# srvk/eesen

Measured on AMD Instinct MI355X. Metric: CTC training frames/sec (whole node), 4x512 BiLSTM, higher is better.
Workload: dtype f32

## Files before the change

### eesen_amd/csrc/kernels.h

```cpp
#pragma once
#include "common.h"

namespace eesen {

struct GemmBound {
  const float* p = nullptr;
  int per_index = 0;
};
void gemm_f32(hipStream_t st, bool a_kc, bool b_kc, int M, int N, int K, float alpha, const float* A, int lda,
              const float* B, int ldb, float beta, float* C, int ldc, const float* bias, float* ws,
              size_t ws_floats, int extra_lds_bytes = 0,
              bool bf16_operands = false,
              GemmBound bound_a = {}, GemmBound bound_b = {});

constexpr int kDefaultGemmMode = 2;
int gemm_mode();
void set_gemm_mode(int mode);
void amax_abs(hipStream_t st, const float* P, long rows, int cols, int ld, float* out);
void amax_abs_accumulate(hipStream_t st, const float* P, long rows, int cols, int ld, float* out);
constexpr int kAmaxBlocks = 512;
void amax_rows_cols(hipStream_t st, const float* P, long rows, int cols, int ld, float* out_rows, float* out_cols, float* ws);

#ifndef EESEN_SHARDS
#define EESEN_SHARDS 8
#endif
constexpr int kShards = EESEN_SHARDS, kShardStride = 32;
constexpr int kCtlHalf = 2048 * kShards;

struct GemmGate {
  const unsigned* cnt;
  unsigned* err;
  int ndir, nz, nblk;
  int T, S;
  int spin_limit;
};
void gemm_f32_nt_gated(hipStream_t st, int M, int N, int K, const float* A, int lda, const float* B, int ldb, float* C,
                       int ldc, const float* bias, const GemmGate& gate, GemmBound bound_a = {}, GemmBound bound_b = {});

struct LstmLayerDev {
  int T, S, H, ndir;
  float* G;
  float* C;
  float* Y;
  float* X = nullptr;
  const float* Wm;
  const float* WmT;
  const float* peep;
  const int* lens;
  const float* rmask = nullptr;
  int drop_mode = 0;
  int s_begin = 0, s_count = 0;
  float* PX = nullptr;
  size_t px_floats = 0;
  int poll_delay = 0;
  int poll_raw = 0;
  unsigned* milestone = nullptr;
  int milestone_step = 0;
  int xcd_map = 1, fwd_mux = 1, bwd_q4 = 1, bwd_ksplit = 1, bwd_mux = 1;
  int fwd_t16_small = 1;
  int fwd_narrow2 = 1;
  int bwd_q4_st8 = 1;
  int fwd_bf16 = 0;
  int fwd_split = 0;
  int fwd_f16 = 0;
  const float* wm_amax = nullptr;
  int bwd_f16 = 0;
  unsigned char* DGH = nullptr;
  float* EX = nullptr;
};
float handoff_flight_ns();
void set_gpu_share(int n);
int gpu_share_value();
void wait_for_word(hipStream_t st, const unsigned* word, unsigned target, unsigned* err, double limit_s = 2.0);
void lstm_fwd_step(hipStream_t st, const LstmLayerDev& L, int step);
void lstm_bwd_step(hipStream_t st, const LstmLayerDev& L, int step, const float* dY, int lddy, float* DG, float* DCF);
void dropout_mask(hipStream_t st, float* out, long rows, int cols, int ld, float p, unsigned long long seed, bool per_column);
void activation_rows(hipStream_t st, bool tanh_, const float* x, int ldx, float* y, int ldy, long rows, int cols);
void activation_diff_rows(hipStream_t st, bool tanh_, const float* y, int ldy, float* d, int ldd, long rows, int cols);
void mul_elements(hipStream_t st, const float* a, int lda, const float* m, int ldm, float* out, int ldo, long rows, int cols);
enum { kRecNone = 0, kRecFwdBf = 1, kRecFwdMux = 2, kRecFwdF32 = 3, kRecBwdQ4 = 4, kRecBwdKsplit = 5, kRecBwdKsplitMux = 6, kRecBwdGeneric = 7 };
struct RecPlan {
  int kind = kRecNone;
  const char* kernel = "";
  int seq_tile = 0;
  int units = 0;
  int windows = 0;
  int grid[3] = {0, 0, 0};
  int wgs = 0;
  int wgs_per_cu = 0;
  int vgprs = 0, lds = 0;
  int free_vgprs = -1;
  int seq_tiles = 1;
  bool one_window = false;
  bool leaves_room = false;
  bool bf16 = false;
  bool light = false;
  size_t need_px = 0, need_ex = 0;
  bool need_dgh = false;
  size_t ctl_words = 0;
  int chunk = 0;
  const void* fn = nullptr;
};
RecPlan lstm_fwd_plan(const LstmLayerDev& L);
RecPlan lstm_bwd_plan(const LstmLayerDev& L);
void lstm_fwd_launch(hipStream_t st, const RecPlan& plan, const LstmLayerDev& L, unsigned* cnt, unsigned* err, int spin_limit,
                     unsigned long long* trace = nullptr, hipEvent_t after_reset = nullptr);
void lstm_bwd_launch(hipStream_t st, const RecPlan& plan, const LstmLayerDev& L, const float* dY, int lddy, float* DG, unsigned* cnt,
                     unsigned* err, int spin_limit, unsigned long long* trace = nullptr);
void lstm_bias_peep_grads(hipStream_t st, const LstmLayerDev& L, const float* DG, float* bias_grad, float* peep_grad,
                          float* ws, size_t ws_floats);
size_t lstm_bias_peep_ws_floats(int T, int S, int H, int ndir);

void col_sums(hipStream_t st, const float* M, int rows, int cols, int ld, float* out, float* ws, size_t ws_floats);
size_t col_sums_ws_floats(int rows, int cols);

void softmax_rows(hipStream_t st, const float* x, int ldx, float* y, int ldy, int rows, int K);
void log_rows(hipStream_t st, const float* in, int ldi, float* out, int ldo, int rows, int K);
void ctc_alpha_beta(hipStream_t st, const float* logp, int ld, int T, int S, int Lpad, const int* labx, const int* lens,
                    const int* lablens, float* alpha, float* beta, float* pzx, int waves = 0);
int ctc_sweep_waves(int Lpad, int waves = 0);
void ctc_best_path(hipStream_t st, const float* scores, int ld, int T, int S, int Lpad, const int* labx, const int* lens,
                   const int* lablens, float* delta, int waves = 0);
void ctc_traceback(hipStream_t st, const float* delta, int T, int S, int Lpad, const int* labx, const int* lens, const int* lablens,
                   int* ali, int* pos, float* score);
void ctc_row_topc(hipStream_t st, const float* scores, int ld, int rows, int K, int S, const int* lens, int Cc, int* cid, float* csc,
                  float* sblank);
struct LmTables;
struct LexTables;
void ctc_prefix_beam(hipStream_t st, const float* scores, int ld, int T, int S, const int* lens, int B, int Cc, const int* cid,
                     const float* csc, const float* sblank, const LmTables* lm, const LexTables* lex, float alpha, float beta, bool use_eos,
                     int* tparent, int* tlabel, int* fnode, int* flen, float* fscore, float* flm, int* count);
void ctc_hyp(hipStream_t st, const int* tparent, const int* tlabel, const int* fnode, const int* flen, const float* fscore, const float* flm,
             const int* count, int T, int S, int B, int N, int* hyp, int* hyp_len, float* score, float* lm_out);
struct WordLexTables;
void ctc_word_beam(hipStream_t st, const float* scores, int ld, int T, int S, const int* lens, int B, int Cc, const int* cid,
                   const float* csc, const float* sblank, const LmTables* lm, const WordLexTables& lex, float alpha, float beta, bool use_eos,
                   int* tparent, int* tlabel, int* tword, int* fnode, int* flen, float* fscore, float* flm, int* fword, int* fnw, int* count);
void ctc_word_hyp(hipStream_t st, const int* tparent, const int* tlabel, const int* tword, const int* fnode, const int* flen, const float* fscore,
                  const float* flm, const int* fword, const int* fnw, const int* count, int T, int S, int B, int N, int* hyp, int* hyp_len,
                  float* score, float* lm_out, int* words, int* ends, int* word_len);
void ctc_error_diff(hipStream_t st, const float* probs, int ld, int T, int S, int K, int Lpad, int Lmax, const int* lens,
                    const int* lablens, const int* labx, const float* alpha, const float* beta,
                    const float* pzx, float* diff, int ldd);
void log_sub_prior(hipStream_t st, float* m, int ld, int rows, int K, bool apply_log, const float* log_prior, float prior_scale);
void row_argmax(hipStream_t st, const float* m, int ld, int rows, int K, int* ids);

struct CeSums {
  double obj;
  long long correct;
};
int ce_eval_blocks(int rows);
void ce_eval(hipStream_t st, const float* y, int ld, int rows, int K, int S, const int* lens, const int* tgt, float* diff,
             int ldd, CeSums* part, CeSums* out);

void sgd_update(hipStream_t st, float* param, float* corr, const float* fresh, long n, float mmt, float lr_coef,
                float max_grad, const unsigned* skip = nullptr, const float* live = nullptr);
void zero_if_set(hipStream_t st, float* p, long n, const unsigned* word);
void adaptive_update(hipStream_t st, float* param, float* corr, const float* fresh, float* accu, long n, float mmt, float lr,
                     float max_grad, float eps, float rho, float one_minus_rho, bool rmsprop, const unsigned* skip = nullptr,
                     const float* live = nullptr);
void tensor_moments(hipStream_t st, const float* base, long rows, int cols, long ld, double* out6, double* ws,
                    int nb = 0, int hf = 0, int hi = 0);
void transpose2d(hipStream_t st, const float* src, int rows, int cols, float* dst);
void copy2d(hipStream_t st, const float* src, int lds, float* dst, int ldd, int rows, int cols);

}
```

### eesen_amd/csrc/net.cpp

```cpp
#include "net.h"

#include <algorithm>
#include <cmath>
#include <cstdio>
#include <cstring>

namespace eesen {


int PhaseTimer::begin(hipStream_t st, int phase) {
  if (!on_) return -1;
  if (used_ == spans_.size()) spans_.emplace_back();
  spans_[used_].phase = phase;
  spans_[used_].a.record(st);
  return (int)used_++;
}
void PhaseTimer::end(hipStream_t st, int idx) {
  if (!on_ || idx < 0) return;
  spans_[idx].b.record(st);
}
void PhaseTimer::collect(float* out, int nphase) {
  for (int i = 0; i < nphase; ++i) out[i] = 0.f;
  for (size_t i = 0; i < used_; ++i) {
    spans_[i].b.wait();
    float ms = 0.f;
    EESEN_HIP_CHECK(hipEventElapsedTime(&ms, spans_[i].a, spans_[i].b));
    if (spans_[i].phase >= 0 && spans_[i].phase < nphase) out[spans_[i].phase] += ms * 1e-3f;
  }
  if (accumulate_) used_ = 0;
}

int PhaseTimer::spans(int* phases, float* secs, int cap) {
  for (size_t i = 0; i < used_ && (int)i < cap; ++i) {
    spans_[i].b.wait();
    float ms = 0.f;
    EESEN_HIP_CHECK(hipEventElapsedTime(&ms, spans_[i].a, spans_[i].b));
    if (phases) phases[i] = spans_[i].phase;
    if (secs) secs[i] = ms * 1e-3f;
  }
  return (int)used_;
}

long Layer::file_params() const {
  if (is_lstm()) return (long)ndir * ((long)4 * Hf * din_f + (long)4 * Hf * Hf + 4 * Hf + 3 * Hf);
  if (kind == EESEN_LAYER_AFFINE) return (long)dout_f * din_f + dout_f;
  return 0;
}

const char* Layer::marker() const {
  switch (kind) {
    case EESEN_LAYER_BILSTM_PARALLEL: return nonparallel ? "<BiLstm>" : "<BiLstmParallel>";
    case EESEN_LAYER_LSTM_PARALLEL: return nonparallel ? "<Lstm>" : "<LstmParallel>";
    case EESEN_LAYER_AFFINE: return "<AffineTransform>";
    case EESEN_LAYER_SOFTMAX: return "<Softmax>";
    case EESEN_LAYER_SIGMOID: return "<Sigmoid>";
    case EESEN_LAYER_TANH: return "<Tanh>";
  }
  return "<Unknown>";
}

template <class F>
static void for_each_param(const Layer& L, F f) {
  long fi = 0;
  if (L.is_lstm()) {
    const int H = L.H, Hf = L.Hf, D = L.din_f, D4 = pad4(L.din);
    for (int dir = 0; dir < L.ndir; ++dir) {
      for (int r = 0; r < 4 * Hf; ++r) {
        const int q = r / Hf, u = r % Hf;
        for (int d = 0; d < D; ++d) f(fi++, L.off_wx + ((size_t)dir * 4 * H + u * 4 + q) * D4 + L.in_col(d));
      }
      for (int r = 0; r < 4 * Hf; ++r) {
        const int q = r / Hf, u = r % Hf;
        for (int k = 0; k < Hf; ++k) f(fi++, L.off_wm + ((size_t)dir * 4 * H + u * 4 + q) * H + k);
      }
      for (int r = 0; r < 4 * Hf; ++r) f(fi++, L.off_bias + (size_t)dir * 4 * H + (r % Hf) * 4 + r / Hf);
      for (int g = 0; g < 3; ++g)
        for (int u = 0; u < Hf; ++u) f(fi++, L.off_peep + ((size_t)dir * 3 + g) * H + u);
    }
  } else if (L.kind == EESEN_LAYER_AFFINE) {
    const int D4 = pad4(L.din);
    for (int r = 0; r < L.dout; ++r)
      for (int d = 0; d < L.din_f; ++d) f(fi++, L.off_w + (size_t)r * D4 + L.in_col(d));
    for (int r = 0; r < L.dout; ++r) f(fi++, L.off_b + r);
  }
}

Net::Net(int dev, void* stream) : device(dev) {
  require_device(dev);
  st = reinterpret_cast<hipStream_t>(stream);
  int lo = 0, hi = 0;
  EESEN_HIP_CHECK(hipDeviceGetStreamPriorityRange(&lo, &hi));
  EESEN_HIP_CHECK(hipStreamCreateWithPriority(&st2.s, hipStreamNonBlocking, lo));
  tn = Tuning::from_env();
  persistent = tn.persistent;
  gate_fwd = tn.gate_fwd >= 0 ? tn.gate_fwd != 0 : gemm_mode() == 0;
  overlap = tn.overlap >= 0 ? tn.overlap != 0 : persistent != 0;
  spin_limit = tn.spin_limit;
  if (tn.trace) {
    trace.reserve(1280);
    EESEN_HIP_CHECK(hipMemset(trace.p, 0, 1280 * sizeof(unsigned long long)));
  }
  ctl.reserve(kCtlWords);
  EESEN_HIP_CHECK(hipMemset(ctl.p, 0, kCtlWords * sizeof(unsigned)));
  {
    constexpr float kFwdNs = 400.f, kBwdNs = 280.f, kBwdSideNs = 420.f, kRefFlightNs = 400.f;
    flight_ns = handoff_flight_ns();
    const float fscale = flight_ns >= 300.f && flight_ns <= 700.f ? 1.f : flight_ns / kRefFlightNs;
    auto ticks = [&](float ns) { return std::min(300, std::max(0, (int)std::lround(fscale * ns / 10.f))); };
    delay_fwd = ticks(kFwdNs); delay_bwd = ticks(kBwdNs); delay_bwd_side = ticks(kBwdSideNs);
    if (const char* e = tn.poll_ns) {
      int a = -1, b2 = -1;
      if (sscanf(e, "%d,%d", &a, &b2) == 2) { delay_fwd = a / 10; delay_bwd = delay_bwd_side = b2 / 10; poll_raw = 1; }
    }
    if (tn.print_flight)
      fprintf(stderr, "eesen_hip: increment flight %.0f ns; first-poll delays forward %d0, backward %d0 (beside side-stream GEMMs %d0) ns\n", flight_ns, delay_fwd, delay_bwd, delay_bwd_side);
  }
}

Net::~Net() {
  (void)hipSetDevice(device);
  (void)hipStreamSynchronize(st);
  for (StatGuard* g : guards) {
    (void)hipStreamSynchronize(g->st);
    g->word = nullptr;
    g->net = nullptr;
  }
  if (trace.p) {
    std::vector<unsigned long long> h(1280);
    if (hipMemcpy(h.data(), trace.p, h.size() * 8, hipMemcpyDeviceToHost) == hipSuccess)
      for (int pass = 0; pass < 2; ++pass) {
        double seg[5] = {0, 0, 0, 0, 0};
        int n = 0;
        for (int s = 8; s < 120; ++s) {
          const unsigned long long* a = h.data() + pass * 640 + s * 5;
          if (!a[0] || !a[5]) continue;
          seg[0] += (double)(a[1] - a[0]); seg[1] += (double)(a[2] - a[1]); seg[2] += (double)(a[3] - a[2]);
          seg[3] += (double)(a[4] - a[3]); seg[4] += (double)(a[5] - a[4]);
          ++n;
        }
        if (n) fprintf(stderr, "EESEN_TRACE %s: wait %.0f | A-load+MFMA+reduce %.0f | epilogue %.0f | drain+barrier %.0f | publish->next %.0f ticks/step (%d steps)\n",
                       pass ? "bwd" : "fwd", seg[0] / n, seg[1] / n, seg[2] / n, seg[3] / n, seg[4] / n, n);
      }
  }
  if (st2) (void)hipStreamSynchronize(st2);
}

void StatGuard::hook(Net* n, int device, hipStream_t stream, const char* entry_point) {
  if (n && !(n->device == device && n->st == stream))
    throw Error(EESEN_ERR_INVALID, std::string(entry_point) + ": the loss object and the Net must live on the same device and stream");
  unhook();
  if (!n || !n->ctl.p) return;
  word = n->ctl.p + kCtlWords - 1;
  net = n;
  st = stream;
  n->guards.push_back(this);
}

void StatGuard::unhook() {
  if (net) net->guards.erase(std::remove(net->guards.begin(), net->guards.end(), this), net->guards.end());
  word = nullptr;
  net = nullptr;
}

void StatGuard::note_dropped(const char* what) {
  if (dropped++ == 0 || dropped % 100 == 0)
    fprintf(stderr, "WARNING (eesen_hip) %s statistics of a minibatch computed from a timed-out forward pass were dropped (%ld so far)\n", what, dropped);
}

void Net::sync() {
  EESEN_HIP_CHECK(hipSetDevice(device));
  EESEN_HIP_CHECK(hipStreamSynchronize(st));
  wait_buckets_host();
  comm_check_alive(comm);
  check_device_error(true);
}

void Net::check_device_error(bool consumer) {
  if (!ctl.p) return;
  unsigned e = 0;
  EESEN_HIP_CHECK(hipMemcpy(&e, ctl.p + kCtlWords - 1, sizeof(unsigned), hipMemcpyDeviceToHost));
  if (!e) { steps_since_clean = 0; return; }
  EESEN_HIP_CHECK(hipStreamSynchronize(st));
  EESEN_HIP_CHECK(hipMemset(ctl.p + kCtlWords - 1, 0, sizeof(unsigned)));
  const bool only_waiter = e == 2 && tn.fwd_mid;
  if (only_waiter) tn.fwd_mid = 0;
  else { persistent = 0; gate_fwd = false; overlap = false; }
  ++recoveries;
  const int lost = std::max(1, steps_since_clean);
  steps_since_clean = 0;
  const bool rerun = consumer && propagated && input.p && rows > 0;
  const char* what = comm ? "contributed a ZERO gradient to the data-parallel sum (the ranks' models stay identical)" : "were NOT applied";
  if (only_waiter)
    fprintf(stderr, "WARNING (eesen_hip) the side stream's wait for a forward-recurrence milestone gave up (kernels serialised by a tool?): "
                    "%d minibatch(es) in flight %s%s; continuing without the early input GEMM (EESEN_FWD_MID=0)\n", lost, what,
            rerun ? " and the last forward pass is re-run" : "");
  else
    fprintf(stderr, "WARNING (eesen_hip) a persistent recurrence kernel gave up waiting for a peer workgroup (GPU shared or preempted?): "
                    "%d minibatch(es) in flight %s%s; continuing with the one-launch-per-step kernels\n", lost, what,
            rerun ? " and the last forward pass is re-run" : "");
  if (rerun) {
    forward_pass();
    EESEN_HIP_CHECK(hipStreamSynchronize(st));
  }
}

void Net::arm_device_error_poll() {
  if (!ctl.p) return;
  if (!err_pin.p) *static_cast<unsigned*>(err_pin.reserve(sizeof(unsigned))) = 0;
  EESEN_HIP_CHECK(hipMemcpyAsync(err_pin.p, ctl.p + kCtlWords - 1, sizeof(unsigned), hipMemcpyDeviceToHost, st));
  err_pin.used(st);
  err_armed = true;
}

void Net::poll_device_error() {
  if (!err_armed || !err_pin.ev.query()) return;
  err_armed = false;
  if (*err_pin.as<unsigned>()) check_device_error(false);
  else steps_since_clean = 0;
}

void Net::add_layer(int kind, int din, int dout, float coef, float max_grad) {
  EESEN_REQUIRE(!finalized, EESEN_ERR_STATE, "net already finalized");
  EESEN_REQUIRE(din > 0 && dout > 0, EESEN_ERR_INVALID, "layer dimensions must be positive");
  const Layer* prev = layers.empty() ? nullptr : &layers.back();
  if (prev)
    EESEN_REQUIRE(prev->dout_f == din, EESEN_ERR_INVALID, "Dimensionality mismatch between consecutive layers");
  Layer L;
  L.kind = kind; L.coef = coef; L.max_grad = max_grad;
  L.din_f = din; L.dout_f = dout;
  L.din = prev ? prev->dout : din;
  if (prev) { L.in_nb = prev->out_nb; L.in_hf = prev->out_hf; L.in_hi = prev->out_hi; }
  L.dout = dout;
  const char* sees_pad = "directly on an LSTM layer whose cell count per direction is not a multiple of 4 is not supported: it would see the "
                         "zero cells the library pads such a layer with";
  switch (kind) {
    case EESEN_LAYER_BILSTM_PARALLEL:
      EESEN_REQUIRE(dout % 2 == 0, EESEN_ERR_INVALID, "<CellDim> of a BiLstm layer must be even");
      L.ndir = 2; L.Hf = dout / 2;
      break;
    case EESEN_LAYER_LSTM_PARALLEL:
      L.ndir = 1; L.Hf = dout;
      break;
    case EESEN_LAYER_AFFINE:
      break;
    case EESEN_LAYER_SOFTMAX:
      EESEN_REQUIRE(din == dout, EESEN_ERR_INVALID, "Softmax needs InputDim == OutputDim");
      if (L.in_nb) throw Error(EESEN_ERR_INVALID, std::string("a <Softmax> ") + sees_pad);
      break;
    case EESEN_LAYER_SIGMOID:
    case EESEN_LAYER_TANH:
      EESEN_REQUIRE(din == dout, EESEN_ERR_INVALID, "an activation layer needs InputDim == OutputDim");
      if (L.in_nb && kind == EESEN_LAYER_SIGMOID) throw Error(EESEN_ERR_INVALID, std::string("a <Sigmoid> ") + sees_pad + " (sigmoid(0) = 1/2)");
      L.dout = L.din;
      L.out_nb = L.in_nb; L.out_hf = L.in_hf; L.out_hi = L.in_hi;
      break;
    default:
      throw Error(EESEN_ERR_INVALID, "unsupported layer kind " + std::to_string(kind));
  }
  if (L.is_lstm()) {
    L.H = pad4(L.Hf);
    L.dout = L.ndir * L.H;
    if (L.H != L.Hf) { L.out_nb = L.ndir; L.out_hf = L.Hf; L.out_hi = L.H; }
  }
  layers.push_back(std::move(L));
}

void Net::finalize() {
  EESEN_REQUIRE(!finalized, EESEN_ERR_STATE, "net already finalized");
  EESEN_REQUIRE(!layers.empty(), EESEN_ERR_INVALID, "empty net");
  EESEN_HIP_CHECK(hipSetDevice(device));
  size_t off = 0;
  for (Layer& L : layers) {
    L.p_off = off;
    size_t n = 0;
    if (L.is_lstm()) {
      const size_t H = L.H, D4 = pad4(L.din), nd = L.ndir;
      L.off_wx = n;   n += nd * 4 * H * D4;
      L.off_bias = n; n += nd * 4 * H;
      L.off_wm = n;   n += nd * 4 * H * H;
      L.off_peep = n; n += nd * 3 * H;
      L.WmT.reserve(nd * H * 4 * H);
    } else if (L.kind == EESEN_LAYER_AFFINE) {
      L.off_w = n; n += (size_t)L.dout * pad4(L.din);
      L.off_b = n; n += pad4(L.dout);
    }
    L.p_n = (n + 3) & ~(size_t)3;
    off += L.p_n;
  }
  P = off;
  if (P) {
    params.reserve(P); corr.reserve(P); fresh.reserve(P + kLiveWords);
    EESEN_HIP_CHECK(hipMemsetAsync(params.p, 0, P * sizeof(float), st));
    EESEN_HIP_CHECK(hipMemsetAsync(corr.p, 0, P * sizeof(float), st));
    EESEN_HIP_CHECK(hipMemsetAsync(fresh.p, 0, (P + kLiveWords) * sizeof(float), st));
  }
  if (tn.overlap < 0)
    for (const Layer& L : layers)
      if (L.is_lstm() && L.H > 512) overlap = false;
  amax.reserve(1 + layers.size());
  EESEN_HIP_CHECK(hipMemsetAsync(amax.p, 0, amax.cap * sizeof(float), st));
  EESEN_HIP_CHECK(hipMemsetD32Async(reinterpret_cast<hipDeviceptr_t>(amax.p), 0x3f800000, 1, st));
  finalized = true;
  refresh_derived();
  sync();
}

void Net::measure(const float* Pm, long nrows, int cols, int ld, DevBuf<float>& out_rows, DevBuf<float>& out_cols) {
  out_rows.reserve((size_t)nrows);
  out_cols.reserve((size_t)cols);
  amax_ws.reserve((size_t)kAmaxBlocks * std::min(16384, (cols + 3) & ~3));
  amax_rows_cols(st, Pm, nrows, cols, ld, out_rows.p, out_cols.p, amax_ws.p);
}
bool Net::x_is_bounded(int li) const {
  if (li == 0) return false;
  const Layer& Pv = layers[li - 1];
  return (Pv.is_lstm() && !Pv.cur_fwd_drop) || Pv.is_activation() || Pv.kind == EESEN_LAYER_SOFTMAX;
}
void Net::ensure_weight_amax() {
  const bool mode2 = gemm_mode() == 2;
  const bool need_w = mode2 && !wamax_valid;
  if (wm_valid && !need_w) return;
  if (!wm_valid) EESEN_HIP_CHECK(hipMemsetAsync(am_wm(0), 0, layers.size() * sizeof(float), st));
  for (size_t li = 0; li < layers.size(); ++li) {
    Layer& L = layers[li];
    if (L.is_lstm()) {
      if (need_w) measure(params.p + L.p_off + L.off_wx, (long)L.ndir * 4 * L.H, pad4(L.din), pad4(L.din), L.bw.rows, L.bw.cols);
      if (!wm_valid) amax_abs_accumulate(st, params.p + L.p_off + L.off_wm, (long)L.ndir * 4 * L.H, L.H, L.H, am_wm((int)li));
    } else if (L.kind == EESEN_LAYER_AFFINE && need_w) measure(params.p + L.p_off + L.off_w, L.dout, pad4(L.din), pad4(L.din), L.bw.rows, L.bw.cols);
  }
  wm_valid = true;
  if (mode2) wamax_valid = true;
}

long Net::num_params() const {
  long n = 0;
  for (const Layer& L : layers) n += L.file_params();
  return n;
}

void Net::init_accu() {
  if (accu_init) return;
  accu.reserve(P);
  EESEN_HIP_CHECK(hipMemsetAsync(accu.p, 0, P * sizeof(float), st));
  accu_init = true;
}

void Net::refresh_derived() {
  wamax_valid = wm_valid = false;
  for (Layer& L : layers)
    if (L.is_lstm())
      for (int dir = 0; dir < L.ndir; ++dir)
        transpose2d(st, params.p + L.p_off + L.off_wm + (size_t)dir * 4 * L.H * L.H, 4 * L.H, L.H,
                    L.WmT.p + (size_t)dir * L.H * 4 * L.H);
}

int Net::tensor_moments(int which, int layer, double* out6_host, int cap_tensors) {
  EESEN_REQUIRE(finalized, EESEN_ERR_STATE, "net not finalized");
  EESEN_REQUIRE(layer >= 0 && layer < (int)layers.size(), EESEN_ERR_INVALID, "layer index out of range");
  EESEN_REQUIRE(which >= 0 && which <= 2, EESEN_ERR_INVALID, "which: 0 parameters, 1 momentum buffers, 2 accumulators");
  const Layer& L = layers[layer];
  struct Region { size_t off; long rows; int cols; long ld; int nb, hf, hi; };
  std::vector<Region> reg;
  if (L.is_lstm()) {
    const int H = L.H, Hf = L.Hf, D4 = pad4(L.din);
    for (int dir = 0; dir < L.ndir; ++dir) {
      reg.push_back({L.off_wx + (size_t)dir * 4 * H * D4, 4L * Hf, L.din_f, D4, L.in_nb, L.in_hf, L.in_hi});
      reg.push_back({L.off_wm + (size_t)dir * 4 * H * H, 4L * Hf, Hf, H, 0, 0, 0});
      reg.push_back({L.off_bias + (size_t)dir * 4 * H, 1, 4 * Hf, 4L * H, 0, 0, 0});
      for (int g = 0; g < 3; ++g) reg.push_back({L.off_peep + ((size_t)dir * 3 + g) * H, 1, Hf, H, 0, 0, 0});
    }
  } else if (L.kind == EESEN_LAYER_AFFINE) {
    reg.push_back({L.off_w, L.dout, L.din_f, pad4(L.din), L.in_nb, L.in_hf, L.in_hi});
    reg.push_back({L.off_b, 1, L.dout, L.dout, 0, 0, 0});
  }
  const int n = (int)reg.size();
  if (!out6_host || n == 0) return n;
  EESEN_REQUIRE(cap_tensors >= n, EESEN_ERR_INVALID, "moments buffer too small");
  EESEN_HIP_CHECK(hipSetDevice(device));
  if (which == 2) init_accu();
  sync();
  const float* base = (which == 0 ? params.p : which == 1 ? corr.p : accu.p) + L.p_off;
  DevBuf<double> d;
  d.reserve((size_t)n * 6 + 8);
  for (int i = 0; i < n; ++i)
    eesen::tensor_moments(st, base + reg[i].off, reg[i].rows, reg[i].cols, reg[i].ld, d.p + (size_t)i * 6, d.p + (size_t)n * 6, reg[i].nb, reg[i].hf, reg[i].hi);
  EESEN_HIP_CHECK(hipStreamSynchronize(st));
  EESEN_HIP_CHECK(hipMemcpy(out6_host, d.p, (size_t)n * 6 * sizeof(double), hipMemcpyDeviceToHost));
  return n;
}

static void upload_flat(Net& net, DevBuf<float>& dst, const float* host, long n) {
  EESEN_REQUIRE(net.finalized, EESEN_ERR_STATE, "net not finalized");
  EESEN_REQUIRE(n == net.num_params(), EESEN_ERR_INVALID, "parameter count mismatch");
  EESEN_HIP_CHECK(hipSetDevice(net.device));
  std::vector<float> h(net.P, 0.f);
  long base = 0;
  for (const Layer& L : net.layers) {
    for_each_param(L, [&](long fi, size_t io) { h[L.p_off + io] = host[base + fi]; });
    base += L.file_params();
  }
  net.sync();
  if (net.P) EESEN_HIP_CHECK(hipMemcpy(dst.p, h.data(), net.P * sizeof(float), hipMemcpyHostToDevice));
}

void Net::set_params(const float* host, long n) {
  upload_flat(*this, params, host, n);
  refresh_derived();
  sync();
}

void Net::set_accu(const float* host, long n) {
  init_accu();
  upload_flat(*this, accu, host, n);
}

void Net::get_flat(const DevBuf<float>& buf, float* host, long n) {
  EESEN_REQUIRE(finalized, EESEN_ERR_STATE, "net not finalized");
  EESEN_REQUIRE(n == num_params(), EESEN_ERR_INVALID, "parameter count mismatch");
  sync();
  std::vector<float> h(P);
  if (P) EESEN_HIP_CHECK(hipMemcpy(h.data(), buf.p, P * sizeof(float), hipMemcpyDeviceToHost));
  long base = 0;
  for (const Layer& L : layers) {
    for_each_param(L, [&](long fi, size_t io) { host[base + fi] = h[L.p_off + io]; });
    base += L.file_params();
  }
}

void Net::set_seq_lengths(const int* l, int s) {
  EESEN_REQUIRE(s > 0, EESEN_ERR_INVALID, "need at least one sequence");
  EESEN_HIP_CHECK(hipSetDevice(device));
  lens.assign(l, l + s);
  for (int v : lens) EESEN_REQUIRE(v >= 0, EESEN_ERR_INVALID, "negative sequence length");
  poll_device_error();
  lens_d.reserve(s);
  int* pinned = static_cast<int*>(lens_pin.reserve(s * sizeof(int), std::max<size_t>(64, (size_t)s * 2) * sizeof(int)));
  std::copy(lens.begin(), lens.end(), pinned);
  EESEN_HIP_CHECK(hipMemcpyAsync(lens_d.p, pinned, s * sizeof(int), hipMemcpyHostToDevice, st));
  lens_pin.used(st);
  S = s;
  propagated = false;
}

static LstmLayerDev lstm_view(const Net& net, const Layer& L, int T) {
  LstmLayerDev d;
  d.T = T; d.S = net.S; d.H = L.H; d.ndir = L.ndir;
  d.G = L.G.p; d.C = L.C.p; d.Y = L.Y.p;
  d.X = L.X.p;
  d.Wm = net.params.p + L.p_off + L.off_wm;
  d.WmT = L.WmT.p;
  d.peep = net.params.p + L.p_off + L.off_peep;
  d.lens = net.lens_d.p;
  d.rmask = L.cur_drop_mode ? L.rmask.p : nullptr;
  d.drop_mode = L.cur_drop_mode;
  d.fwd_bf16 = net.fwd_bf16_rec ? 1 : 0;
  d.fwd_split = net.tn.fwd_split;
  d.fwd_f16 = net.tn.fwd_f16 && net.tn.fwd_split;
  d.bwd_f16 = net.tn.bwd_f16 && net.tn.fwd_split;
  d.wm_amax = net.amax.p ? const_cast<Net&>(net).am_wm((int)(&L - net.layers.data())) : nullptr;
  d.xcd_map = net.tn.xcd_map; d.fwd_mux = net.tn.fwd_mux; d.bwd_q4 = net.tn.bwd_q4; d.bwd_q4_st8 = net.tn.bwd_q4_st8; d.fwd_narrow2 = net.tn.fwd_narrow2; d.fwd_t16_small = net.tn.fwd_t16_small; d.bwd_ksplit = net.tn.bwd_ksplit; d.bwd_mux = net.tn.bwd_mux;
  return d;
}

void Net::set_layer_dropout(int layer, const float* nine) {
  EESEN_REQUIRE(layer >= 0 && layer < (int)layers.size(), EESEN_ERR_INVALID, "layer index out of range");
  Layer& L = layers[layer];
  bool any = false;
  for (int k = 0; k < 9; ++k) any |= nine[k] != 0.f;
  EESEN_REQUIRE(!any || L.kind == EESEN_LAYER_BILSTM_PARALLEL, EESEN_ERR_INVALID, "dropout options exist on BiLstm layers only");
  EESEN_REQUIRE(nine[0] >= 0.f && nine[0] < 1.f && nine[7] >= 0.f && nine[7] < 1.f, EESEN_ERR_INVALID, "dropout factor outside [0, 1)");
  for (int k = 0; k < 9; ++k) L.drop[k] = (k == 0 || k == 7) ? nine[k] : (nine[k] != 0.f ? 1.f : 0.f);
}

void Net::get_layer_dropout(int layer, float* nine) const {
  EESEN_REQUIRE(layer >= 0 && layer < (int)layers.size(), EESEN_ERR_INVALID, "layer index out of range");
  for (int k = 0; k < 9; ++k) nine[k] = layers[layer].drop[k];
}

static void widen_mask(const Layer& L, const float* src, long n, std::vector<float>& dst, const char* what) {
  dst.clear();
  if (!src) return;
  const long wf = (long)L.ndir * L.Hf, wi = (long)L.ndir * L.H;
  EESEN_REQUIRE(n > 0 && n % wf == 0, EESEN_ERR_INVALID, std::string(what) + ": the float count is not a multiple of the layer's ndir * H columns");
  if (wf == wi) { dst.assign(src, src + n); return; }
  const long rows = n / wf;
  dst.assign((size_t)rows * wi, 0.f);
  for (long r = 0; r < rows; ++r)
    for (int d = 0; d < L.ndir; ++d)
      std::copy(src + r * wf + (long)d * L.Hf, src + r * wf + (long)(d + 1) * L.Hf, dst.begin() + r * wi + (long)d * L.H);
}

void Net::set_dropout_masks(int layer, const float* fwd, long fwd_n, const float* rec, int rec_rows, long rec_n, int coin) {
  EESEN_REQUIRE(layer >= 0 && layer < (int)layers.size() && layers[layer].is_lstm(), EESEN_ERR_INVALID, "not an LSTM layer");
  Layer& L = layers[layer];
  if (rec) EESEN_REQUIRE(rec_rows > 0 && rec_n == (long)rec_rows * L.ndir * L.Hf, EESEN_ERR_INVALID, "recurrent mask: rec_floats must be rec_rows x ndir * H");
  widen_mask(L, fwd, fwd ? fwd_n : 0, L.inj_fmask, "forward mask");
  widen_mask(L, rec, rec ? rec_n : 0, L.inj_rmask, "recurrent mask");
  L.inj_rmask_rows = rec ? rec_rows : 0;
  L.inj_coin = coin;
}

void Net::get_dropout_masks(int layer, float* fwd_host, float* rec_host, int* info4) {
  EESEN_REQUIRE(layer >= 0 && layer < (int)layers.size() && layers[layer].is_lstm(), EESEN_ERR_INVALID, "not an LSTM layer");
  EESEN_REQUIRE(propagated, EESEN_ERR_STATE, "no Propagate yet");
  Layer& L = layers[layer];
  EESEN_HIP_CHECK(hipSetDevice(device));
  sync();
  const size_t ldY = (size_t)L.ndir * L.H, wf = (size_t)L.ndir * L.Hf;
  auto fetch = [&](float* host, const float* dev, size_t nrows) {
    if (wf == ldY) { EESEN_HIP_CHECK(hipMemcpy(host, dev, nrows * ldY * sizeof(float), hipMemcpyDeviceToHost)); return; }
    std::vector<float> tmp(nrows * ldY);
    EESEN_HIP_CHECK(hipMemcpy(tmp.data(), dev, tmp.size() * sizeof(float), hipMemcpyDeviceToHost));
    for (size_t r = 0; r < nrows; ++r)
      for (int d = 0; d < L.ndir; ++d)
        std::copy(tmp.begin() + r * ldY + (size_t)d * L.H, tmp.begin() + r * ldY + (size_t)d * L.H + L.Hf, host + r * wf + (size_t)d * L.Hf);
  };
  if (fwd_host && L.cur_fwd_drop) fetch(fwd_host, L.fmask.p, (size_t)rows);
  if (rec_host && L.cur_drop_mode) fetch(rec_host, L.rmask.p, (size_t)(T + 2) * S);
  if (info4) { info4[0] = L.cur_fwd_drop; info4[1] = L.cur_drop_mode; info4[2] = L.cur_twiddle_coin; info4[3] = (int)wf; }
}

static void prepare_dropout(Net& net, Layer& L) {
  L.cur_fwd_drop = false; L.cur_drop_mode = 0; L.cur_twiddle_coin = false;
  const bool want = net.in_train && L.has_dropout();
  if (!want) { L.inj_fmask.clear(); L.inj_rmask.clear(); L.inj_rmask_rows = 0; L.inj_coin = -1; return; }
  const float fwd_p = L.drop[0], rec_p = L.drop[7];
  const bool fw_seq = L.drop[2] != 0.f, rec_step = L.drop[3] != 0.f, rec_seq = L.drop[4] != 0.f;
  const bool rnndrop = L.drop[5] != 0.f, nml = L.drop[6] != 0.f, twiddle = L.drop[8] != 0.f;
  const int T = net.T, S = net.S, ldY = L.ndir * L.H;
  bool coin = false;
  if (twiddle) {
    if (L.inj_coin >= 0) coin = L.inj_coin != 0;
    else {
      unsigned long long z = net.drop_seed + (++net.drop_counter) * 0x9E3779B97F4A7C15ull;
      z = (z ^ (z >> 30)) * 0xBF58476D1CE4E5B9ull; z = (z ^ (z >> 27)) * 0x94D049BB133111EBull; z ^= z >> 31;
      coin = (z >> 63) != 0;
    }
  }
  L.cur_twiddle_coin = coin;
  const bool rec = (rnndrop || nml) && (!twiddle || !coin);
  const bool fwd = fwd_p > 0.f && (!twiddle || coin);
  if (rec) {
    EESEN_REQUIRE(rec_step != rec_seq, EESEN_ERR_INVALID,
                  "recurrent dropout needs exactly one of RecurrentTimeStepDropout / RecurrentSequenceDropout (bilstm-layer.h:102-113)");
    EESEN_REQUIRE(!(rnndrop && nml), EESEN_ERR_INVALID, "RNNDrop and NoMemLossDropout are mutually exclusive");
    const long mrows = (long)(T + 2) * S;
    L.rmask.reserve((size_t)mrows * ldY);
    if (!L.inj_rmask.empty()) {
      EESEN_REQUIRE((L.inj_rmask_rows == mrows || L.inj_rmask_rows == S) && (long)L.inj_rmask.size() == (long)L.inj_rmask_rows * ldY,
                    EESEN_ERR_INVALID, "injected recurrent mask has the wrong shape");
      const size_t chunk = (size_t)L.inj_rmask_rows * ldY;
      for (long r0 = 0; r0 < mrows; r0 += L.inj_rmask_rows)
        EESEN_HIP_CHECK(hipMemcpyAsync(L.rmask.p + (size_t)r0 * ldY, L.inj_rmask.data(), chunk * sizeof(float), hipMemcpyHostToDevice, net.st));
      EESEN_HIP_CHECK(hipStreamSynchronize(net.st));
    } else {
      dropout_mask(net.st, L.rmask.p, mrows, ldY, ldY, rec_p, net.drop_seed + (++net.drop_counter) * 0x632BE59BD9B4E019ull, rec_seq);
    }
    L.cur_drop_mode = rnndrop ? 2 : 1;
  }
  if (fwd) {
    L.fmask.reserve((size_t)net.rows * ldY);
    L.Yd.reserve((size_t)net.rows * ldY);
    if (!L.inj_fmask.empty()) {
      EESEN_REQUIRE((long)L.inj_fmask.size() == (long)net.rows * ldY, EESEN_ERR_INVALID, "injected forward mask has the wrong shape");
      EESEN_HIP_CHECK(hipMemcpyAsync(L.fmask.p, L.inj_fmask.data(), L.inj_fmask.size() * sizeof(float), hipMemcpyHostToDevice, net.st));
      EESEN_HIP_CHECK(hipStreamSynchronize(net.st));
    } else {
      dropout_mask(net.st, L.fmask.p, net.rows, ldY, ldY, fwd_p, net.drop_seed + (++net.drop_counter) * 0x632BE59BD9B4E019ull, fw_seq);
    }
    L.cur_fwd_drop = true;
  }
  L.inj_fmask.clear(); L.inj_rmask.clear(); L.inj_rmask_rows = 0; L.inj_coin = -1;
}

void Net::propagate(const float* in, int nrows, int ld, bool is_device) {
  EESEN_REQUIRE(finalized, EESEN_ERR_STATE, "net not finalized");
  EESEN_REQUIRE(S > 0, EESEN_ERR_STATE, "SetSeqLengths must precede Propagate");
  EESEN_REQUIRE(nrows > 0 && nrows % S == 0, EESEN_ERR_INVALID, "row count must be a positive multiple of the sequence count");
  const int D = layers[0].din, D4 = pad4(D);
  EESEN_REQUIRE(ld >= D, EESEN_ERR_INVALID, "input leading dimension smaller than InputDim");
  EESEN_HIP_CHECK(hipSetDevice(device));
  rows = nrows;
  T = rows / S;
  for (int v : lens) EESEN_REQUIRE(v <= T, EESEN_ERR_INVALID, "sequence length exceeds the number of frames");
  timer.reset();

  if (input.reserve((size_t)rows * D4) || D4 != D) EESEN_HIP_CHECK(hipMemsetAsync(input.p, 0, (size_t)rows * D4 * sizeof(float), st));
  if (is_device) {
    EESEN_HIP_CHECK(hipMemcpy2DAsync(input.p, (size_t)D4 * sizeof(float), in, (size_t)ld * sizeof(float), (size_t)D * sizeof(float), rows,
                                     hipMemcpyDeviceToDevice, st));
  } else {
    PinBuf& hs = in_stage[in_stage_idx++ & 1];
    const size_t bytes = (size_t)rows * D * sizeof(float);
    float* staged = static_cast<float*>(hs.reserve(bytes, bytes + bytes / 4));
    for (int r = 0; r < rows; ++r) std::memcpy(staged + (size_t)r * D, in + (size_t)r * ld, (size_t)D * sizeof(float));
    EESEN_HIP_CHECK(hipMemcpy2DAsync(input.p, (size_t)D4 * sizeof(float), staged, (size_t)D * sizeof(float), (size_t)D * sizeof(float), rows,
                                     hipMemcpyHostToDevice, st));
    hs.used(st);
  }
  forward_pass();
}

void Net::forward_pass() {
  const float* x = input.p;
  int ldx = pad4(layers[0].din);
  ++steps_since_clean;
  info_fwd_persistent = info_lstm_layers = info_fwd_bf16 = 0;
  bool g_gated = false;
  int gated_rows = 0;
  int mid_r0 = 0, mid_r1 = 0;
  const bool half = gemm_mode() == 2;
  ensure_weight_amax();
  amx_valid = half;
  for (Layer& L : layers) {
    const int li_ = (int)(&L - layers.data());
    GemmBound x_amax, w_amax;
    if (half && L.trainable()) {
      if (x_is_bounded(li_)) x_amax = bound_one();
      else { measure(x, rows, L.din, ldx, L.bx.rows, L.bx.cols); x_amax = GemmBound{L.bx.rows.p, 1}; }
      w_amax = GemmBound{L.bw.rows.p, 1};
    }
    if (L.is_lstm()) {
      const int H = L.H, nd = L.ndir, ldY = nd * H, ldG = nd * 4 * H;
      L.G.reserve((size_t)rows * ldG);
      const size_t state = (size_t)(T + 2) * S * ldY;
      L.C.reserve(state);
      L.Y.reserve(state);
      if (persistent && H % 32 == 0) L.X.reserve((size_t)T * nd * ((S + 15) / 16) * (size_t)(H / 32) * 768);
      const size_t blk = (size_t)S * ldY * sizeof(float);
      EESEN_HIP_CHECK(hipMemsetAsync(L.C.p, 0, blk, st));
      EESEN_HIP_CHECK(hipMemsetAsync(L.Y.p, 0, blk, st));
      EESEN_HIP_CHECK(hipMemsetAsync(L.C.p + (size_t)(T + 1) * S * ldY, 0, blk, st));
      EESEN_HIP_CHECK(hipMemsetAsync(L.Y.p + (size_t)(T + 1) * S * ldY, 0, blk, st));
      prepare_dropout(*this, L);
      if (g_gated) {
        if (gated_rows < rows) {
          const int ti_ = timer.begin(st, 0);
          gemm_f32(st, true, true, rows - gated_rows, ldG, L.din, 1.f, x + (size_t)gated_rows * ldx, ldx, params.p + L.p_off + L.off_wx,
                   pad4(L.din), 0.f, L.G.p + (size_t)gated_rows * ldG, ldG, params.p + L.p_off + L.off_bias, nullptr, 0, 0, fwd_bf16, x_amax, w_amax);
          timer.end(st, ti_);
        }
        EESEN_HIP_CHECK(hipStreamWaitEvent(st, ev_gate_done, 0));
        g_gated = false;
      } else if (mid_r1 > mid_r0) {
        const int ti_ = timer.begin(st, 0);
        const int parts[2][2] = {{0, mid_r0}, {mid_r1, rows}};
        for (const auto& pr : parts)
          if (pr[1] > pr[0])
            gemm_f32(st, true, true, pr[1] - pr[0], ldG, L.din, 1.f, x + (size_t)pr[0] * ldx, ldx, params.p + L.p_off + L.off_wx, pad4(L.din),
                     0.f, L.G.p + (size_t)pr[0] * ldG, ldG, params.p + L.p_off + L.off_bias, nullptr, 0, 0, fwd_bf16, x_amax, w_amax);
        timer.end(st, ti_);
        EESEN_HIP_CHECK(hipStreamWaitEvent(st, ev_gate_done, 0));
        mid_r0 = mid_r1 = 0;
      } else {
        const int ti_ = timer.begin(st, 0);
        gemm_f32(st, true, true, rows, ldG, L.din, 1.f, x, ldx, params.p + L.p_off + L.off_wx, pad4(L.din), 0.f, L.G.p, ldG,
                 params.p + L.p_off + L.off_bias, nullptr, 0, 0, fwd_bf16, x_amax, w_amax);
        timer.end(st, ti_);
      }
      Layer* nxt = (&L - layers.data()) + 1 < (long)layers.size() ? &layers[(&L - layers.data()) + 1] : nullptr;
      LstmLayerDev v = lstm_view(*this, L, T);
      const RecPlan fp = persistent ? lstm_fwd_plan(v) : RecPlan{};
      const bool pers = fp.kind != kRecNone;
      const bool plan_gate = pers && overlap && gate_fwd && !fwd_bf16 && !L.cur_fwd_drop && fp.units <= 8 && nxt && nxt->is_lstm() && T >= 2 && rows >= 128 &&
                             fp.one_window &&
                             (nxt->ndir * 4 * nxt->H) % 128 == 0 && ldY % 16 == 0 && nd * fp.seq_tiles * kShards <= 64;
      const int mile_step = (3 * T) / 4;
      const bool plan_mid = pers && overlap && tn.fwd_mid && !plan_gate && !L.cur_fwd_drop && fp.leaves_room && nd == 2 && nxt && nxt->is_lstm() &&
                            T >= 32 && mile_step + 1 < T && fp.one_window;
      { const int ti_ = timer.begin(st, 1);
      v.poll_delay = delay_fwd;
      v.poll_raw = poll_raw;
      if (plan_mid) {
        mile.reserve(32);
        EESEN_HIP_CHECK(hipMemsetAsync(mile.p, 0, 2 * sizeof(unsigned), st));
        EESEN_HIP_CHECK(hipEventRecord(ev_gate_reset, st));
        v.milestone = mile.p;
        v.milestone_step = mile_step;
      }
      if (pers) lstm_fwd_launch(st, fp, v, ctl.p, ctl.p + kCtlWords - 1, spin_limit, trace.p, plan_gate ? ev_gate_reset.get() : nullptr);
      else
        for (int step = 0; step < T; ++step) lstm_fwd_step(st, v, step);
      info_fwd_persistent += pers ? 1 : 0;
      info_fwd_bf16 += fp.bf16 ? 1 : 0;
      ++info_lstm_layers;
      check_launch("lstm_fwd");
      timer.end(st, ti_);
      if (pers && plan_gate) {
        const int ldG2 = nxt->ndir * 4 * nxt->H;
        nxt->G.reserve((size_t)rows * ldG2);
        EESEN_HIP_CHECK(hipStreamWaitEvent(st2, ev_gate_reset, 0));
        const int tj_ = timer.begin(st2, 0);
        GemmGate gate{ctl.p, ctl.p + kCtlWords - 1, nd, fp.seq_tiles, fp.grid[0], T, S, spin_limit};
        gated_rows = rows / 128 * 128;
        gemm_f32_nt_gated(st2, gated_rows, ldG2, ldY, L.Y.p + (size_t)S * ldY, ldY, params.p + nxt->p_off + nxt->off_wx, pad4(nxt->din),
                          nxt->G.p, ldG2, params.p + nxt->p_off + nxt->off_bias, gate, half ? bound_one() : GemmBound{}, half ? GemmBound{nxt->bw.rows.p, 1} : GemmBound{});
        timer.end(st2, tj_);
        EESEN_HIP_CHECK(hipEventRecord(ev_gate_done, st2));
        g_gated = true;
      }
      if (plan_mid) {
        EESEN_HIP_CHECK(hipMemsetD32Async(reinterpret_cast<hipDeviceptr_t>(mile.p + 1), 1, 1, st));
        const int ldG2 = nxt->ndir * 4 * nxt->H;
        nxt->G.reserve((size_t)rows * ldG2);
        mid_r0 = ((T - 1 - mile_step) * S + 255) / 256 * 256;
        mid_r1 = (mile_step + 1) * S / 256 * 256;
        if (mid_r1 <= mid_r0) mid_r0 = mid_r1 = 0;
      }
      if (plan_mid && mid_r1 > mid_r0) {
        const int ldG2 = nxt->ndir * 4 * nxt->H;
        EESEN_HIP_CHECK(hipStreamWaitEvent(st2, ev_gate_reset, 0));
        wait_for_word(st2, mile.p + 1, 1u, ctl.p + kCtlWords - 1, 2.0 * std::max(1.0, T / 1000.0) * std::max(1.0, spin_limit / 400000.0));
        const int tj_ = timer.begin(st2, 0);
        gemm_f32(st2, true, true, mid_r1 - mid_r0, ldG2, nxt->din, 1.f, L.Y.p + (size_t)S * ldY + (size_t)mid_r0 * ldY, ldY,
                 params.p + nxt->p_off + nxt->off_wx, pad4(nxt->din), 0.f, nxt->G.p + (size_t)mid_r0 * ldG2, ldG2,
                 params.p + nxt->p_off + nxt->off_bias, nullptr, 0,  64, fwd_bf16,
                 half ? bound_one() : GemmBound{}, half ? GemmBound{nxt->bw.rows.p, 1} : GemmBound{});
        timer.end(st2, tj_);
        EESEN_HIP_CHECK(hipEventRecord(ev_gate_done, st2));
      } }
      if (L.cur_fwd_drop)
        mul_elements(st, L.Y.p + (size_t)S * ldY, ldY, L.fmask.p, ldY, L.Yd.p, ldY, rows, ldY);
      x = L.output(S);
      ldx = ldY;
    } else if (L.kind == EESEN_LAYER_AFFINE) {
      const int ldo = pad4(L.dout);
      if (L.out.reserve((size_t)rows * ldo)) EESEN_HIP_CHECK(hipMemsetAsync(L.out.p, 0, L.out.cap * sizeof(float), st));
      { const int ti_ = timer.begin(st, 2);
      gemm_f32(st, true, true, rows, L.dout, L.din, 1.f, x, ldx, params.p + L.p_off + L.off_w, pad4(L.din), 0.f, L.out.p, ldo,
               params.p + L.p_off + L.off_b, nullptr, 0, 0, fwd_bf16, x_amax, w_amax);
      timer.end(st, ti_); }
      x = L.out.p;
      ldx = ldo;
    } else if (L.is_activation()) {
      const int ldo = pad4(L.dout);
      if (L.out.reserve((size_t)rows * ldo)) EESEN_HIP_CHECK(hipMemsetAsync(L.out.p, 0, L.out.cap * sizeof(float), st));
      { const int ti_ = timer.begin(st, 2);
      activation_rows(st, L.kind == EESEN_LAYER_TANH, x, ldx, L.out.p, ldo, rows, L.dout);
      timer.end(st, ti_); }
      x = L.out.p;
      ldx = ldo;
    } else {
      const int ldo = pad4(L.dout);
      if (L.out.reserve((size_t)rows * ldo)) EESEN_HIP_CHECK(hipMemsetAsync(L.out.p, 0, L.out.cap * sizeof(float), st));
      { const int ti_ = timer.begin(st, 2);
      softmax_rows(st, x, ldx, L.out.p, ldo, rows, L.dout);
      timer.end(st, ti_); }
      x = L.out.p;
      ldx = ldo;
    }
  }
  out_ptr = x;
  out_cols = layers.back().dout;
  out_ld = ldx;
  if (const Layer& Lb = layers.back(); Lb.out_nb) {
    const int ldo = pad4(Lb.dout_f);
    if (out_f.reserve((size_t)rows * ldo) && ldo != Lb.dout_f) EESEN_HIP_CHECK(hipMemsetAsync(out_f.p, 0, out_f.cap * sizeof(float), st));
    for (int b = 0; b < Lb.out_nb; ++b) copy2d(st, x + (size_t)b * Lb.out_hi, ldx, out_f.p + (size_t)b * Lb.out_hf, ldo, rows, Lb.out_hf);
    out_ptr = out_f.p; out_cols = Lb.dout_f; out_ld = ldo;
  }
  propagated = true;
  if (persistent) arm_device_error_poll();
}

void Net::backpropagate(const float* out_diff, int ldd, float* in_diff, int ldi) {
  bucket_log.clear();
  deferred_buckets.clear();
  try {
    backpropagate_impl(out_diff, ldd, in_diff, ldi);
  } catch (...) {
    fail_step_buckets();
    throw;
  }
}

void Net::backpropagate_impl(const float* out_diff, int ldd, float* in_diff, int ldi) {
  EESEN_REQUIRE(propagated, EESEN_ERR_STATE, "Backpropagate needs a preceding Propagate");
  EESEN_HIP_CHECK(hipSetDevice(device));
  int maxdim = 0, max_g = 0, max_y = 0;
  size_t need_ws = 0;
  for (const Layer& L : layers) {
    maxdim = std::max(maxdim, std::max(pad4(L.din), pad4(L.dout)));
    if (L.is_lstm()) {
      max_g = std::max(max_g, L.ndir * 4 * L.H);
      max_y = std::max(max_y, L.ndir * L.H);
      need_ws = std::max(need_ws, lstm_bias_peep_ws_floats(T, S, L.H, L.ndir));
    }
    need_ws = std::max(need_ws, col_sums_ws_floats(rows, L.dout));
  }
  need_ws = std::max(need_ws, (size_t)16 << 20);
  ws.reserve(need_ws);
  ws_floats = need_ws;
  dA.reserve((size_t)rows * maxdim);
  dB.reserve((size_t)rows * maxdim);
  if (max_g) {
    DGb[0].reserve((size_t)rows * max_g);
    DGb[1].reserve((size_t)rows * max_g);
  }
  if (max_y) DCF.reserve((size_t)S * max_y);
  ws2.reserve(need_ws);
  int dg_slot = 0;
  bool side_pending[2] = {false, false};
  deferred_buckets.clear();
  const std::vector<RecPlan> bwd = bwd_plans(T);
  const bool overlap = overlap_for_minibatch(bwd);
  exchange_deferred = comm && exchange_deferred_for_minibatch(bwd);
  bucket_log.clear();
  info_bwd_persistent = 0;
  live_valid = comm != nullptr;
  if (comm) {
    comm_check_alive(comm);
    EESEN_HIP_CHECK(hipMemsetD32Async(reinterpret_cast<hipDeviceptr_t>(fresh.p + P), 0x3f800000, 1, st));
  }

  const int Kout = layers.back().dout;
  float* d = dA.p;
  int ld_d = pad4(Kout);
  float* dn = dB.p;
  const bool half = gemm_mode() == 2;
  ensure_weight_amax();
  auto x_cols = [&](int li) -> GemmBound {
    if (!half || !amx_valid) return GemmBound{};
    return x_is_bounded(li) ? bound_one() : GemmBound{layers[li].bx.cols.p, 1};
  };
  if (const Layer& Lb = layers.back(); Lb.out_nb) {
    EESEN_HIP_CHECK(hipMemsetAsync(d, 0, (size_t)rows * ld_d * sizeof(float), st));
    for (int b = 0; b < Lb.out_nb; ++b) copy2d(st, out_diff + (size_t)b * Lb.out_hf, ldd, d + (size_t)b * Lb.out_hi, ld_d, rows, Lb.out_hf);
  } else {
    if (ld_d != Kout) EESEN_HIP_CHECK(hipMemsetAsync(d, 0, (size_t)rows * ld_d * sizeof(float), st));
    copy2d(st, out_diff, ldd, d, ld_d, rows, Kout);
  }

  for (int li = (int)layers.size() - 1; li >= 0; --li) {
    Layer& L = layers[li];
    const float* x;
    int ldx;
    if (li == 0) { x = input.p; ldx = pad4(L.din); }
    else {
      const Layer& Pv = layers[li - 1];
      if (Pv.is_lstm()) { ldx = Pv.ndir * Pv.H; x = Pv.output(S); }
      else { ldx = pad4(Pv.dout); x = Pv.out.p; }
    }
    const bool want_in = li > 0 || in_diff != nullptr;
    const int ld_n = pad4(L.din);
    float* fr = fresh.p + L.p_off;
    if (L.kind == EESEN_LAYER_SOFTMAX) {
      continue;
    } else if (L.is_activation()) {
      { const int ti_ = timer.begin(st, 4);
      activation_diff_rows(st, L.kind == EESEN_LAYER_TANH, L.out.p, pad4(L.dout), d, ld_d, rows, L.dout);
      timer.end(st, ti_); }
      continue;
    } else if (L.kind == EESEN_LAYER_AFFINE) {
      { const int ti_ = timer.begin(st, 4);
      if (half) measure(d, rows, L.dout, ld_d, L.bd.rows, L.bd.cols);
      if (want_in) {
        if (ld_n != L.din) EESEN_HIP_CHECK(hipMemsetAsync(dn, 0, (size_t)rows * ld_n * sizeof(float), st));
        gemm_f32(st, true, false, rows, L.din, L.dout, 1.f, d, ld_d, params.p + L.p_off + L.off_w, pad4(L.din), 0.f, dn, ld_n,
                 nullptr, nullptr, 0, 0, false, half ? GemmBound{L.bd.rows.p, 1} : GemmBound{}, half ? GemmBound{L.bw.cols.p, 1} : GemmBound{});
      }
      gemm_f32(st, false, false, L.dout, L.din, rows, 1.f, d, ld_d, x, ldx, 0.f, fr + L.off_w, pad4(L.din), nullptr, ws.p, ws_floats, 0, false,
               half ? GemmBound{L.bd.cols.p, 1} : GemmBound{}, x_cols(li));
      col_sums(st, d, rows, L.dout, ld_d, fr + L.off_b, ws.p, ws_floats);
      timer.end(st, ti_); }
      bucket_allreduce(li, st);
    } else {
      const int H = L.H, nd = L.ndir, ldG = nd * 4 * H, ldY = nd * H;
      LstmLayerDev v = lstm_view(*this, L, T);
      v.poll_delay = overlap ? delay_bwd_side : delay_bwd;
      v.poll_raw = poll_raw;
      const RecPlan& bp = bwd[li];
      if (bp.need_px) { bwd_px.reserve(bp.need_px); v.PX = bwd_px.p; v.px_floats = bwd_px.cap; }
      if (bp.need_dgh) {
        bwd_dgh.reserve((size_t)rows * ldG);
        bwd_ex.reserve(bp.need_ex);
        v.DGH = reinterpret_cast<unsigned char*>(bwd_dgh.p);
        v.EX = bwd_ex.p;
      }
      EESEN_REQUIRE(in_train || !L.has_dropout(), EESEN_ERR_STATE, "Can't backpropagate a dropout layer in test mode (bilstm-parallel-layer.h:425)");
      if (L.cur_fwd_drop) mul_elements(st, d, ld_d, L.fmask.p, ldY, d, ld_d, rows, ldY);
      float* DGl = DGb[dg_slot].p;
      if (side_pending[dg_slot]) {
        EESEN_HIP_CHECK(hipStreamWaitEvent(st, ev_grad[dg_slot], 0));
        side_pending[dg_slot] = false;
      }
      { const int ti_ = timer.begin(st, 3);
      if (bp.kind != kRecNone) {
        lstm_bwd_launch(st, bp, v, d, ld_d, DGl, ctl.p + kCtlHalf, ctl.p + kCtlWords - 1, spin_limit, trace.p ? trace.p + 640 : nullptr);
        ++info_bwd_persistent;
      } else
        for (int step = 0; step < T; ++step) lstm_bwd_step(st, v, step, d, ld_d, DGl, DCF.p);
      check_launch("lstm_bwd");
      timer.end(st, ti_); }
      if (half) { const int ti_ = timer.begin(st, 4); measure(DGl, rows, ldG, ldG, L.bd.rows, L.bd.cols); timer.end(st, ti_); }
      EESEN_HIP_CHECK(hipEventRecord(ev_rec, st));
      if (want_in) {
        const int ti_ = timer.begin(st, 4);
        if (ld_n != L.din) EESEN_HIP_CHECK(hipMemsetAsync(dn, 0, (size_t)rows * ld_n * sizeof(float), st));
        gemm_f32(st, true, false, rows, L.din, ldG, 1.f, DGl, ldG, params.p + L.p_off + L.off_wx, pad4(L.din), 0.f, dn, ld_n,
                 nullptr, nullptr, 0, 0, false, half ? GemmBound{L.bd.rows.p, 1} : GemmBound{}, half ? GemmBound{L.bw.cols.p, 1} : GemmBound{});
        timer.end(st, ti_);
        EESEN_HIP_CHECK(hipEventRecord(ev_rec, st));
      }
      hipStream_t sg = overlap ? st2 : st;
      const int side_lds_env = (tn.side_lds_kb >= 0 ? tn.side_lds_kb : (gemm_mode() >= 1 ? 48 : 32)) * 1024;
      bool lstm_below = false;
      for (int lj = 0; lj < li; ++lj) lstm_below |= layers[lj].is_lstm();
      const int side_lds = overlap && lstm_below ? side_lds_env : 0;
      if (overlap) EESEN_HIP_CHECK(hipStreamWaitEvent(st2, ev_rec, 0));
      { const int ti_ = timer.begin(sg, 4);
      gemm_f32(sg, false, false, ldG, L.din, rows, 1.f, DGl, ldG, x, ldx, 0.f, fr + L.off_wx, pad4(L.din), nullptr, ws2.p, need_ws, side_lds, false,
               half ? GemmBound{L.bd.cols.p, 1} : GemmBound{}, x_cols(li));
      for (int dir = 0; dir < nd; ++dir)
        gemm_f32(sg, false, false, 4 * H, H, rows, 1.f, DGl + (size_t)dir * 4 * H, ldG,
                 L.Y.p + (size_t)(dir == 0 ? 0 : 2 * S) * ldY + (size_t)dir * H, ldY, 0.f,
                 fr + L.off_wm + (size_t)dir * 4 * H * H, H, nullptr, ws2.p, need_ws, side_lds, false,
                 half ? GemmBound{L.bd.cols.p + (size_t)dir * 4 * H, 1} : GemmBound{}, half ? bound_one() : GemmBound{});
      lstm_bias_peep_grads(sg, v, DGl, fr + L.off_bias, fr + L.off_peep, ws2.p, need_ws);
      timer.end(sg, ti_); }
      bucket_allreduce(li, sg);
      if (overlap) {
        EESEN_HIP_CHECK(hipEventRecord(ev_grad[dg_slot], st2));
        side_pending[dg_slot] = true;
      }
      dg_slot ^= 1;
    }
    if (want_in) {
      std::swap(d, dn);
      ld_d = ld_n;
    }
  }
  if (in_diff) copy2d(st, d, ld_d, in_diff, ldi, rows, layers[0].din);
  flush_deferred_buckets();
  for (int k = 0; k < 2; ++k)
    if (side_pending[k]) EESEN_HIP_CHECK(hipStreamWaitEvent(st, ev_grad[k], 0));
}

std::vector<RecPlan> Net::bwd_plans(int T) const {
  std::vector<RecPlan> plans(layers.size());
  for (size_t li = 0; li < layers.size(); ++li)
    if (persistent && layers[li].is_lstm()) plans[li] = lstm_bwd_plan(lstm_view(*this, layers[li], T));
  return plans;
}
bool Net::overlap_for_minibatch(const std::vector<RecPlan>& bwd) const {
  bool ov = overlap;
  if (ov && tn.overlap < 0 && persistent)
    for (size_t li = 0; li < layers.size(); ++li)
      if (const Layer& L = layers[li]; L.is_lstm() && L.H > 320 && L.H <= 512 && S > 32 && !bwd[li].light) ov = false;
  return ov;
}
bool Net::exchange_deferred_for_minibatch(const std::vector<RecPlan>& bwd) const {
  if (tn.comm_defer >= 0) return tn.comm_defer != 0;
  if (!persistent) return false;
  for (const RecPlan& bp : bwd)
    if (bp.kind != kRecNone && bp.free_vgprs < kRcclVgprsPerSimdLane) return true;
  return false;
}

std::string Net::plan_string() const {
  EESEN_REQUIRE(finalized, EESEN_ERR_STATE, "net not finalized");
  EESEN_REQUIRE(S > 0, EESEN_ERR_STATE, "call eesen_net_set_seq_lengths first: the plan depends on the minibatch shape");
  EESEN_HIP_CHECK(hipSetDevice(device));
  int T = this->T;
  if (!propagated) { T = 0; for (int v : lens) T = std::max(T, v); }
  auto one = [](const RecPlan& P) {
    char b[512];
    if (P.kind == kRecNone) { snprintf(b, sizeof(b), "{\"kernel\": \"per-step kernels (lstm.hip)\", \"persistent\": false}"); return std::string(b); }
    snprintf(b, sizeof(b), "{\"kernel\": \"%s\", \"persistent\": true, \"sequences_per_workgroup\": %d, \"units_per_workgroup\": %d, \"grid\": [%d, %d, %d], "
             "\"workgroups\": %d, \"workgroups_per_cu\": %d, \"launches\": %d, \"vgprs\": %d, \"lds_bytes\": %d, \"free_vgprs_per_simd_lane\": %d}",
             P.kernel, P.seq_tile, P.units, P.grid[0], P.grid[1], P.grid[2], P.wgs, P.wgs_per_cu, P.windows, P.vgprs, P.lds, P.free_vgprs);
    return std::string(b);
  };
  const std::vector<RecPlan> bwd = bwd_plans(T);
  std::string o = "{\"T\": " + std::to_string(T) + ", \"S\": " + std::to_string(S) + ", \"persistent\": " + (persistent ? "true" : "false") + ", \"layers\": [";
  bool first = true;
  for (size_t li = 0; li < layers.size(); ++li) {
    const Layer& L = layers[li];
    if (!L.is_lstm()) continue;
    const RecPlan fp = persistent && T >= 1 ? lstm_fwd_plan(lstm_view(*this, L, T)) : RecPlan{}, &bp = bwd[li];
    o += std::string(first ? "" : ", ") + "{\"layer\": " + std::to_string(li) + ", \"cells\": " + std::to_string(L.H) + ", \"directions\": " + std::to_string(L.ndir) +
         ", \"forward\": " + one(fp) + ", \"backward\": " + one(bp) + "}";
    first = false;
  }
  const bool ov = overlap_for_minibatch(bwd);
  o += std::string("], \"weight_gradient_gemms\": \"") + (ov ? "side stream, under the next-lower recurrence" : "main stream, serial") + "\"";
  o += std::string(", \"gemm_arithmetic\": \"") + (gemm_mode() == 2 ? "two fp16 planes, three products (fp32-class)" : gemm_mode() == 1 ? "3-way bf16 split (fp32-class)" : "f32-input MFMA") + "\"";
  o += std::string(", \"exchange\": ") + (comm ? (exchange_deferred_for_minibatch(bwd) ? "\"deferred: every bucket behind the backward pass's last recurrence\""
                                                                                      : "\"overlapped: each bucket as soon as its layer's gradients are enqueued\"") : "null");
  o += std::string(", \"exchange_rule\": \"") + (tn.comm_defer >= 0 ? "EESEN_COMM_DEFER" : "auto: deferred when a persistent backward grid leaves < 256 registers per SIMD lane") + "\"";
  o += ", \"gpu_share\": " + std::to_string(gpu_share_value()) + "}";
  return o;
}

void Net::update() {
  EESEN_REQUIRE(finalized, EESEN_ERR_STATE, "net not finalized");
  EESEN_HIP_CHECK(hipSetDevice(device));
  const unsigned* skip = persistent && !grads_sanitized ? ctl.p + kCtlWords - 1 : nullptr;
  const float* live = comm && live_valid ? fresh.p + P : nullptr;
  comm_check_alive(comm);
  { const int ti_ = timer.begin(st, 5);
  for (int li = (int)layers.size() - 1; li >= 0; --li) {
    Layer& L = layers[li];
    if (L.p_n) {
      if (comm && li < (int)bucket_pending.size() && bucket_pending[li]) {
        const int tw_ = timer.begin(st, 7);
        EESEN_HIP_CHECK(hipStreamWaitEvent(st, ev_bucket[li], 0));
        timer.end(st, tw_);
        bucket_pending[li] = 0;
      }
      if (rule == 0) {
        sgd_update(st, params.p + L.p_off, corr.p + L.p_off, fresh.p + L.p_off, (long)L.p_n, mmt, lr * L.coef, L.max_grad, skip, live);
      } else {
        init_accu();
        adaptive_update(st, params.p + L.p_off, corr.p + L.p_off, fresh.p + L.p_off, accu.p + L.p_off, (long)L.p_n, mmt, lr,
                        L.max_grad, ada_eps, rms_rho, rms_one_minus_rho, rule == 2, skip, live);
      }
    }
  }
  refresh_derived();
  timer.end(st, ti_); }
  grads_sanitized = false;
  live_valid = false;
  if (persistent) arm_device_error_poll();
}

}
```

### eesen_amd/csrc/net.h

```cpp
#pragma once
#include <string>
#include <vector>

#include "kernels.h"
#include "lex.h"
#include "lm.h"
#include "tuning.h"

namespace eesen {

inline int pad4(int x) { return (x + 3) & ~3; }
constexpr size_t kCtlWords = 2 * kCtlHalf + 32;

struct Layer {
  int kind = 0, din = 0, dout = 0;
  float coef = 1.f, max_grad = 0.f;
  size_t p_off = 0, p_n = 0;
  int H = 0, ndir = 0;
  int din_f = 0, dout_f = 0, Hf = 0;
  int in_nb = 0, in_hf = 0, in_hi = 0, out_nb = 0, out_hf = 0, out_hi = 0;
  int in_col(int d) const { return in_nb ? (d / in_hf) * in_hi + d % in_hf : d; }
  size_t off_wx = 0, off_bias = 0, off_wm = 0, off_peep = 0;
  DevBuf<float> WmT;
  DevBuf<float> G, C, Y;
  DevBuf<float> X;
  size_t off_w = 0, off_b = 0;
  DevBuf<float> out;
  struct Bounds { DevBuf<float> rows, cols; } bw, bx, bd;
  float drop[9] = {0, 0, 0, 0, 0, 0, 0, 0, 0};
  bool has_dropout() const { return drop[0] > 0.f || drop[5] != 0.f || drop[6] != 0.f; }
  DevBuf<float> fmask;
  DevBuf<float> rmask;
  DevBuf<float> Yd;
  bool cur_fwd_drop = false;
  int cur_drop_mode = 0;
  bool cur_twiddle_coin = false;
  std::vector<float> inj_fmask, inj_rmask;
  int inj_rmask_rows = 0, inj_coin = -1;
  const float* output(int S) const { return cur_fwd_drop ? Yd.p : Y.p + (size_t)S * ndir * H; }
  bool is_lstm() const { return kind == EESEN_LAYER_LSTM_PARALLEL || kind == EESEN_LAYER_BILSTM_PARALLEL; }
  bool nonparallel = false;
  bool is_activation() const { return kind == EESEN_LAYER_SIGMOID || kind == EESEN_LAYER_TANH; }
  bool trainable() const { return is_lstm() || kind == EESEN_LAYER_AFFINE; }
  long file_params() const;
  const char* marker() const;
};

class PhaseTimer {
 public:
  void enable(bool on) { on_ = on; }
  bool enabled() const { return on_; }
  void set_accumulate(bool a) { accumulate_ = a; used_ = 0; }
  void reset() { if (!accumulate_) used_ = 0; }
  int begin(hipStream_t st, int phase);
  void end(hipStream_t st, int idx);
  void collect(float* out, int nphase);
  int spans(int* phases, float* secs, int cap);
 private:
  struct Span { DevEvent a{true}, b{true}; int phase = 0; };
  std::vector<Span> spans_;
  size_t used_ = 0;
  bool on_ = false, accumulate_ = false;
};

struct Comm;
void comm_check_alive(const Comm* c);
constexpr size_t kLiveWords = 4;
constexpr int kRcclVgprsPerSimdLane = 256;

struct StatGuard {
  const unsigned* word = nullptr;
  struct Net* net = nullptr;
  long dropped = 0;
  hipStream_t st = nullptr;
  StatGuard() = default;
  StatGuard(const StatGuard&) = delete;
  StatGuard& operator=(const StatGuard&) = delete;
  ~StatGuard() { unhook(); }
  void hook(struct Net* n, int device, hipStream_t stream, const char* entry_point);
  void unhook();
  void note_dropped(const char* what);
};

struct Net {
  int device = 0;
  hipStream_t st = nullptr;
  std::vector<Layer> layers;
  bool finalized = false;
  size_t P = 0;
  DevBuf<float> params, corr, fresh;
  float lr = 0.f, mmt = 0.f;
  int rule = 0;
  float ada_eps = 1e-6f, rms_rho = 0.9f, rms_one_minus_rho = 0.1f;
  DevBuf<float> accu;
  bool accu_init = false;
  void init_accu();
  void set_accu(const float* host, long n);
  std::vector<int> lens;
  DevBuf<int> lens_d;
  int T = 0, S = 0, rows = 0;
  bool propagated = false;
  DevBuf<float> input;
  PinBuf in_stage[2];
  unsigned in_stage_idx = 0;
  const float* out_ptr = nullptr;
  int out_cols = 0, out_ld = 0;
  DevBuf<float> out_f;
  DevBuf<float> DGb[2], DCF, dA, dB, ws, ws2;
  DevBuf<float> bwd_px;
  DevBuf<float> bwd_dgh, bwd_ex;
  DevStream st2;
  DevEvent ev_rec, ev_grad[2];
  bool overlap = true;
  DevEvent ev_gate_reset, ev_gate_done;
  DevBuf<unsigned> mile;
  bool gate_fwd = true;
  bool fwd_bf16 = false;
  bool fwd_bf16_rec = false;
  int info_fwd_bf16 = 0;
  DevBuf<unsigned> ctl;
  Tuning tn;
  int persistent = 1;
  int info_fwd_persistent = 0, info_bwd_persistent = 0, info_lstm_layers = 0;
  int spin_limit = 400000;
  float flight_ns = 0.f;
  int delay_fwd = 61, delay_bwd = 43, delay_bwd_side = 64, poll_raw = 0;
  int recoveries = 0;
  DevBuf<unsigned long long> trace;
  void check_device_error(bool consumer);
  int steps_since_clean = 0;
  PinBuf lens_pin, err_pin;
  bool err_armed = false;
  void poll_device_error();
  void arm_device_error_poll();
  bool in_train = true;
  unsigned long long drop_seed = 777, drop_counter = 0;
  void set_train_mode(bool train) { in_train = train; }
  void set_layer_dropout(int layer, const float* nine);
  void get_layer_dropout(int layer, float* nine) const;
  void set_dropout_masks(int layer, const float* fwd, long fwd_n, const float* rec, int rec_rows, long rec_n, int coin);
  void get_dropout_masks(int layer, float* fwd_host, float* rec_host, int* info4);
  size_t ws_floats = 0;
  DevBuf<float> amax, amax_ws;
  bool wamax_valid = false, wm_valid = false;
  bool amx_valid = false;
  float* am_wm(int li) { return amax.p + 1 + li; }
  GemmBound bound_one() const { return GemmBound{amax.p, 0}; }
  bool x_is_bounded(int li) const;
  void measure(const float* P, long rows, int cols, int ld, DevBuf<float>& out_rows, DevBuf<float>& out_cols);
  void ensure_weight_amax();
  PhaseTimer timer;
  Comm* comm = nullptr;
  std::vector<DevEvent> ev_ready, ev_bucket;
  std::vector<char> bucket_pending;
  std::vector<int> deferred_buckets;
  bool exchange_deferred = false;
  std::vector<RecPlan> bwd_plans(int T) const;
  bool overlap_for_minibatch(const std::vector<RecPlan>& bwd) const;
  bool exchange_deferred_for_minibatch(const std::vector<RecPlan>& bwd) const;
  std::string plan_string() const;
  DevEvent ev_bwd_done;
  void issue_bucket(int li);
  void fail_step_buckets() noexcept;
  void flush_deferred_buckets();
  std::vector<StatGuard*> guards;
  bool grads_sanitized = false;
  bool live_valid = false;
  std::vector<int> bucket_log;
  PinBuf live_pin;
  void set_comm(Comm* c);
  int top_trainable() const;
  int live_ranks();
  void bucket_allreduce(int li, hipStream_t producer);
  void wait_buckets_host();
  void backpropagate_zero();
  void allreduce_grads(Comm* c);

  Net(int device, void* stream);
  ~Net();
  void add_layer(int kind, int din, int dout, float coef, float max_grad);
  void finalize();
  long num_params() const;
  void set_params(const float* host, long n);
  void get_flat(const DevBuf<float>& buf, float* host, long n);
  void set_seq_lengths(const int* lens, int S);
  void propagate(const float* in, int rows, int ld, bool is_device);
  void forward_pass();
  void backpropagate(const float* out_diff, int ldd, float* in_diff, int ldi);
  void backpropagate_impl(const float* out_diff, int ldd, float* in_diff, int ldi);
  void update();
  void refresh_derived();
  int tensor_moments(int which, int layer, double* out6_host, int cap_tensors);
  void read(const std::string& path);
  void write(const std::string& path, bool binary);
  void sync();
};

inline void* loss_slot(PinBuf& pin, size_t bytes) { return pin.reserve(bytes, std::max<size_t>(bytes * 2, 4096)); }

struct Ctc {
  int device = 0;
  hipStream_t st = nullptr;
  DevBuf<float> logp, alpha, beta, pzx_d;
  DevBuf<int> labx, ids_d, ali_d;
  std::vector<int> last_lens;
  int last_T = 0, last_S = 0, last_Lpad = 0, last_Lprime = 0;
  int sweep_waves = 0;
  double obj_sum = 0;
  long sequences = 0, frames = 0, err_tokens = 0, ref_tokens = 0;
  DevEvent ev[4] = {DevEvent(true), DevEvent(true), DevEvent(true), DevEvent(true)};
  PhaseTimer timer;
  DevEvent aev[4] = {DevEvent(true), DevEvent(true), DevEvent(true), DevEvent(true)};
  PhaseTimer align_timer;
  PinBuf align_pin;
  DevBuf<float> dec_f;
  DevBuf<int> dec_i, dec_trie, dec_out;
  DevEvent dev[4] = {DevEvent(true), DevEvent(true), DevEvent(true), DevEvent(true)};
  PhaseTimer decode_timer;
  PinBuf decode_pin;
  int dec_rows = 0, dec_S = 0, dec_C = 0;
  std::vector<int> dec_lens;
  DevBuf<int> lm_i;
  DevBuf<float> lm_f;
  LmTables lm_tab{};
  unsigned long long lm_serial = 0;
  DevBuf<int> lex_i;
  LexTables lex_tab{};
  WordLexTables word_tab{};
  unsigned long long lex_serial = 0;
  PinBuf stage[2];
  unsigned stage_idx = 0;
  struct PendingPzx { PinBuf pin; int S = 0; long nframes = 0; bool active = false; } ppzx[2];
  struct PendingErr { PinBuf pin, probs; int S = 0, K = 0, rows = 0; bool active = false, with_probs = false, guarded = false; std::vector<int> frames, ids, off; } perr[2];
  StatGuard guard;
  std::string seq_out;
  unsigned ppzx_idx = 0, perr_idx = 0;
  void flush_pzx(PendingPzx& q);
  void flush_err(PendingErr& q, int* num_err, int* num_ref);
  void flush();

  Ctc(int device, void* stream);
  ~Ctc();
  void eval_parallel(const int* frame_num_utt, int S, const float* net_out, int rows, int K, int ld, const int* label_ids,
                     const int* label_off, float* diff, int ldd, float* pzx_host);
  void error_rate_mseq(const int* frame_num_utt, int S, const float* net_out, int rows, int K, int ld,
                       const int* label_ids, const int* label_off, int* num_err, int* num_ref);
  void get_alpha_beta(float* alpha_host, float* beta_host, int* Lprime);
  void phase_times(float* out3);
  void align_parallel(const int* frame_num_utt, int S, const float* scores, int rows, int K, int ld, bool is_log, const int* label_ids,
                      const int* label_off, int* ali_host, int* pos_host, float* score_host);
  void align_times(float* out3);
  void decode_parallel(const int* frame_num_utt, int S, const float* scores, int rows, int K, int ld, bool is_log, int beam, int max_classes,
                       int nbest, int* hyp_host, int* hyp_len_host, float* score_host);
  void decode_parallel_lm(const int* frame_num_utt, int S, const float* scores, int rows, int K, int ld, bool is_log, int beam, int max_classes,
                          int nbest, const TokenLm* lm, float lm_weight, float insertion_bonus, bool use_eos, int* hyp_host, int* hyp_len_host,
                          float* score_host, float* lm_score_host);
  void decode_parallel_lex(const int* frame_num_utt, int S, const float* scores, int rows, int K, int ld, bool is_log, int beam, int max_classes,
                           int nbest, const Lexicon* lex, const TokenLm* lm, float lm_weight, float word_bonus, bool use_eos, int* hyp_host,
                           int* hyp_len_host, float* score_host, float* lm_score_host, int* word_host, int* word_len_host);
  void decode_parallel_words(const int* frame_num_utt, int S, const float* scores, int rows, int K, int ld, bool is_log, int beam, int max_classes,
                             int nbest, const Lexicon* lex, const TokenLm* lm, float lm_weight, float word_bonus, bool use_eos, int* hyp_host,
                             int* hyp_len_host, float* score_host, float* lm_score_host, int* word_host, int* word_len_host, int* word_end_host);
  void decode_times(float* out3);
  void get_decode_candidates(int* ids_host, float* scores_host, float* blank_host, int* Cc);
 private:
  struct Lattices { const int *labx, *lens, *lablens; int Lpad, Lprime; };
  Lattices upload_lattices(const int* frame_num_utt, int S, const int* label_ids, const int* label_off);
  void decode_batch(const int* frame_num_utt, int S, const float* scores, int rows, int K, int ld, bool is_log, int beam, int max_classes,
                    int nbest, const Lexicon* lex, const TokenLm* lm, float lm_weight, float insertion_bonus, bool use_eos, int* hyp_host,
                    int* hyp_len_host, float* score_host, float* lm_score_host);
  void upload_lm(const TokenLm& lm);
  void upload_lex(const Lexicon& lex);
};

int edit_distance(const int* ref, int nr, const int* hyp, int nh);

struct CeLoss {
  int device = 0;
  hipStream_t st = nullptr;
  DevBuf<int> tg;
  DevBuf<CeSums> part, res;
  PinBuf stage[2];
  unsigned stage_idx = 0;
  struct Pending { PinBuf pin; int S = 0; long rows = 0; bool active = false; } pend[2];
  unsigned pend_idx = 0;
  double obj = 0, obj_progress = 0;
  long correct = 0, frames = 0, sequences = 0, correct_progress = 0, frames_progress = 0, sequences_progress = 0;
  int report_step = 100;
  std::vector<std::string> progress;
  StatGuard guard;
  DevEvent ev[2] = {DevEvent(true), DevEvent(true)};
  PhaseTimer timer;

  CeLoss(int device, void* stream);
  ~CeLoss();
  void fold(Pending& q, double* obj_out);
  void flush();
  void eval_parallel(const int* frame_num_utt, int S, const float* net_out, int rows, int K, int ld, const int* targets,
                     float* diff, int ldd, double* obj_host);
  std::string report();
  void phase_times(float* out1);
};

}
```

### eesen_amd/csrc/optim.hip

```cpp
#include "kernels.h"

namespace eesen {
namespace {

__global__ __launch_bounds__(256) void sgd_update_kernel(float* __restrict__ param, float* __restrict__ corr,
                                                         const float* __restrict__ fresh, long n, float mmt,
                                                         float lr_coef, float max_grad, const unsigned* __restrict__ skip,
                                                         const float* __restrict__ live) {
  if (skip && *skip) return;
  if (live && *live == 0.f) return;
  const long n4 = n >> 2;
  const long stride = (long)gridDim.x * blockDim.x;
  for (long i = (long)blockIdx.x * blockDim.x + threadIdx.x; i < n4; i += stride) {
    float4 p = reinterpret_cast<float4*>(param)[i];
    float4 c = reinterpret_cast<float4*>(corr)[i];
    const float4 g = reinterpret_cast<const float4*>(fresh)[i];
    c.x = mmt * c.x + g.x; c.y = mmt * c.y + g.y; c.z = mmt * c.z + g.z; c.w = mmt * c.w + g.w;
    if (max_grad > 0.f) {
      c.x = fminf(fmaxf(c.x, -max_grad), max_grad); c.y = fminf(fmaxf(c.y, -max_grad), max_grad);
      c.z = fminf(fmaxf(c.z, -max_grad), max_grad); c.w = fminf(fmaxf(c.w, -max_grad), max_grad);
    }
    p.x -= lr_coef * c.x; p.y -= lr_coef * c.y; p.z -= lr_coef * c.z; p.w -= lr_coef * c.w;
    reinterpret_cast<float4*>(corr)[i] = c;
    reinterpret_cast<float4*>(param)[i] = p;
  }
  for (long i = (n4 << 2) + (long)blockIdx.x * blockDim.x + threadIdx.x; i < n; i += stride) {
    float c = mmt * corr[i] + fresh[i];
    if (max_grad > 0.f) c = fminf(fmaxf(c, -max_grad), max_grad);
    corr[i] = c;
    param[i] -= lr_coef * c;
  }
}

__global__ __launch_bounds__(256) void adaptive_update_kernel(float* __restrict__ param, float* __restrict__ corr,
                                                              const float* __restrict__ fresh, float* __restrict__ accu,
                                                              long n, float mmt, float lr, float max_grad, float eps,
                                                              float rho, float one_minus_rho, int rmsprop,
                                                              const unsigned* __restrict__ skip, const float* __restrict__ live) {
  if (skip && *skip) return;
  if (live && *live == 0.f) return;
  const long stride = (long)gridDim.x * blockDim.x;
  for (long i = (long)blockIdx.x * blockDim.x + threadIdx.x; i < n; i += stride) {
    float c = mmt * corr[i] + fresh[i];
    if (max_grad > 0.f) c = fminf(fmaxf(c, -max_grad), max_grad);
    const float g2 = c * c;
    float a = accu[i];
    a = rmsprop ? (rho * a + one_minus_rho * g2) : (a + g2);
    const float scale = 1.0f / sqrtf(a + eps);
    corr[i] = c;
    accu[i] = a;
    param[i] += -lr * scale * c;
  }
}

__global__ __launch_bounds__(256) void zero_if_set_kernel(float* __restrict__ p, long n, const unsigned* __restrict__ word) {
  if (*word == 0u) return;
  const long stride = (long)gridDim.x * blockDim.x;
  for (long i = (long)blockIdx.x * blockDim.x + threadIdx.x; i < n; i += stride) p[i] = 0.f;
}

__global__ __launch_bounds__(256) void transpose2d_kernel(const float* __restrict__ src, int rows, int cols,
                                                          float* __restrict__ dst) {
  __shared__ float tile[32][33];
  const int tx = threadIdx.x & 31, ty = threadIdx.x >> 5;
  const int c0 = blockIdx.x * 32, r0 = blockIdx.y * 32;
#pragma unroll
  for (int i = 0; i < 32; i += 8) {
    const int r = r0 + ty + i, c = c0 + tx;
    if (r < rows && c < cols) tile[ty + i][tx] = src[(size_t)r * cols + c];
  }
  __syncthreads();
#pragma unroll
  for (int i = 0; i < 32; i += 8) {
    const int c = c0 + ty + i, r = r0 + tx;
    if (r < rows && c < cols) dst[(size_t)c * rows + r] = tile[tx][ty + i];
  }
}

__global__ __launch_bounds__(256) void copy2d_kernel(const float* __restrict__ src, int lds, float* __restrict__ dst,
                                                     int ldd, int rows, int cols) {
  const size_t total = (size_t)rows * cols;
  for (size_t i = (size_t)blockIdx.x * blockDim.x + threadIdx.x; i < total; i += (size_t)gridDim.x * blockDim.x) {
    const size_t r = i / cols, c = i % cols;
    dst[r * ldd + c] = src[r * lds + c];
  }
}

}

void sgd_update(hipStream_t st, float* param, float* corr, const float* fresh, long n, float mmt, float lr_coef,
                float max_grad, const unsigned* skip, const float* live) {
  if (n <= 0) return;
  const int blocks = (int)std::min<long>(cdivl(n / 4 + 1, 256), 2048);
  hipLaunchKernelGGL(sgd_update_kernel, dim3(blocks), dim3(256), 0, st, param, corr, fresh, n, mmt, lr_coef, max_grad, skip, live);
  check_launch("sgd_update");
}

void zero_if_set(hipStream_t st, float* p, long n, const unsigned* word) {
  if (n <= 0 || !word) return;
  hipLaunchKernelGGL(zero_if_set_kernel, dim3(256), dim3(256), 0, st, p, n, word);
  check_launch("zero_if_set");
}

void adaptive_update(hipStream_t st, float* param, float* corr, const float* fresh, float* accu, long n, float mmt, float lr,
                     float max_grad, float eps, float rho, float one_minus_rho, bool rmsprop, const unsigned* skip, const float* live) {
  if (n <= 0) return;
  const int blocks = (int)std::min<long>(cdivl(n, 256), 4096);
  hipLaunchKernelGGL(adaptive_update_kernel, dim3(blocks), dim3(256), 0, st, param, corr, fresh, accu, n, mmt, lr, max_grad, eps,
                     rho, one_minus_rho, rmsprop ? 1 : 0, skip, live);
  check_launch("adaptive_update");
}

void transpose2d(hipStream_t st, const float* src, int rows, int cols, float* dst) {
  hipLaunchKernelGGL(transpose2d_kernel, dim3(cdiv(cols, 32), cdiv(rows, 32)), dim3(256), 0, st, src, rows, cols, dst);
  check_launch("transpose2d");
}

void copy2d(hipStream_t st, const float* src, int lds, float* dst, int ldd, int rows, int cols) {
  if (rows <= 0 || cols <= 0) return;
  const size_t total = (size_t)rows * cols;
  const int blocks = (int)std::min<size_t>((total + 255) / 256, 4096);
  hipLaunchKernelGGL(copy2d_kernel, dim3(blocks), dim3(256), 0, st, src, lds, dst, ldd, rows, cols);
  check_launch("copy2d");
}


namespace {
__device__ __forceinline__ float hash_uniform(unsigned long long seed, unsigned long long idx) {
  unsigned long long z = seed + (idx + 1ull) * 0x9E3779B97F4A7C15ull;
  z = (z ^ (z >> 30)) * 0xBF58476D1CE4E5B9ull;
  z = (z ^ (z >> 27)) * 0x94D049BB133111EBull;
  z ^= z >> 31;
  return (float)(z >> 40) * (1.0f / 16777216.0f);
}
__global__ __launch_bounds__(256) void dropout_mask_kernel(float* __restrict__ out, long rows, int cols, int ld, float p, float scale,
                                                           unsigned long long seed, int per_column) {
  const long n = rows * cols;
  for (long i = (long)blockIdx.x * blockDim.x + threadIdx.x; i < n; i += (long)gridDim.x * blockDim.x) {
    const long r = i / cols;
    const int c = (int)(i % cols);
    const float u = hash_uniform(seed, per_column ? (unsigned long long)c : (unsigned long long)i);
    out[r * ld + c] = (u - p > 0.f) ? scale : 0.f;
  }
}
__global__ __launch_bounds__(256) void mul_elements_kernel(const float* __restrict__ a, int lda, const float* __restrict__ m, int ldm,
                                                           float* __restrict__ out, int ldo, long rows, int cols) {
  const long n = rows * cols;
  for (long i = (long)blockIdx.x * blockDim.x + threadIdx.x; i < n; i += (long)gridDim.x * blockDim.x) {
    const long r = i / cols;
    const int c = (int)(i % cols);
    out[r * ldo + c] = a[r * lda + c] * m[r * ldm + c];
  }
}
template <bool TANH>
__global__ __launch_bounds__(256) void activation_kernel(const float* __restrict__ x, int ldx, float* __restrict__ y, int ldy, long rows, int cols) {
  const long n = rows * cols;
  for (long i = (long)blockIdx.x * blockDim.x + threadIdx.x; i < n; i += (long)gridDim.x * blockDim.x) {
    const long r = i / cols;
    const int c = (int)(i % cols);
    const float v = x[r * ldx + c];
    float o;
    if (TANH) {
      const float e = expf(2.0f * v);
      o = isinf(e) ? 1.0f : (e - 1.0f) / (e + 1.0f);
    } else {
      o = 1.0f / (1.0f + expf(-v));
    }
    y[r * ldy + c] = o;
  }
}
template <bool TANH>
__global__ __launch_bounds__(256) void activation_diff_kernel(const float* __restrict__ y, int ldy, float* __restrict__ d, int ldd, long rows, int cols) {
  const long n = rows * cols;
  for (long i = (long)blockIdx.x * blockDim.x + threadIdx.x; i < n; i += (long)gridDim.x * blockDim.x) {
    const long r = i / cols;
    const int c = (int)(i % cols);
    const float o = y[r * ldy + c];
    d[r * ldd + c] *= TANH ? (1.0f - o * o) : o * (1.0f - o);
  }
}
}

void activation_rows(hipStream_t st, bool tanh_, const float* x, int ldx, float* y, int ldy, long rows, int cols) {
  if (rows <= 0 || cols <= 0) return;
  const int blocks = (int)std::min<long>(cdivl(rows * cols, 256), 256L * 16);
  if (tanh_) hipLaunchKernelGGL(activation_kernel<true>, dim3(blocks), dim3(256), 0, st, x, ldx, y, ldy, rows, cols);
  else hipLaunchKernelGGL(activation_kernel<false>, dim3(blocks), dim3(256), 0, st, x, ldx, y, ldy, rows, cols);
  check_launch("activation_rows");
}

void activation_diff_rows(hipStream_t st, bool tanh_, const float* y, int ldy, float* d, int ldd, long rows, int cols) {
  if (rows <= 0 || cols <= 0) return;
  const int blocks = (int)std::min<long>(cdivl(rows * cols, 256), 256L * 16);
  if (tanh_) hipLaunchKernelGGL(activation_diff_kernel<true>, dim3(blocks), dim3(256), 0, st, y, ldy, d, ldd, rows, cols);
  else hipLaunchKernelGGL(activation_diff_kernel<false>, dim3(blocks), dim3(256), 0, st, y, ldy, d, ldd, rows, cols);
  check_launch("activation_diff_rows");
}

void dropout_mask(hipStream_t st, float* out, long rows, int cols, int ld, float p, unsigned long long seed, bool per_column) {
  if (rows <= 0 || cols <= 0) return;
  const int blocks = (int)std::min<long>(cdivl(rows * cols, 256), 256L * 16);
  hipLaunchKernelGGL(dropout_mask_kernel, dim3(blocks), dim3(256), 0, st, out, rows, cols, ld, p, 1.0f / (1.0f - p), seed, per_column ? 1 : 0);
  check_launch("dropout_mask");
}

void mul_elements(hipStream_t st, const float* a, int lda, const float* m, int ldm, float* out, int ldo, long rows, int cols) {
  if (rows <= 0 || cols <= 0) return;
  const int blocks = (int)std::min<long>(cdivl(rows * cols, 256), 256L * 16);
  hipLaunchKernelGGL(mul_elements_kernel, dim3(blocks), dim3(256), 0, st, a, lda, m, ldm, out, ldo, rows, cols);
  check_launch("mul_elements");
}

namespace {
template <int PASS>
__global__ __launch_bounds__(1024) void tensor_moments_kernel(const float* __restrict__ base, long rows, int cols, long ld,
                                                              double* __restrict__ out6, double* __restrict__ ws, int nb, int hf, int hi) {
  __shared__ double red[4][16];
  const long n = rows * cols;
  const int tid = threadIdx.x, lane = tid & 63, wave = tid >> 6;
  double a = PASS == 0 ? 1e300 : 0.0, b = PASS == 0 ? -1e300 : 0.0, c = 0.0, d = 0.0;
  const double mean = PASS == 1 ? ws[2] / (double)n : 0.0;
  for (long i = tid; i < n; i += 1024) {
    const int cf = (int)(i % cols);
    const double v = (double)base[(i / cols) * ld + (nb ? (cf / hf) * hi + cf % hf : cf)];
    if (PASS == 0) { a = fmin(a, v); b = fmax(b, v); c += v; }
    else { const double e = v - mean, e2 = e * e; a += e2; b += e2 * e; c += e2 * e2; }
  }
  for (int off = 32; off > 0; off >>= 1) {
    const double a2 = __shfl_down(a, off), b2 = __shfl_down(b, off), c2 = __shfl_down(c, off);
    if (PASS == 0) { a = fmin(a, a2); b = fmax(b, b2); c += c2; }
    else { a += a2; b += b2; c += c2; }
  }
  if (lane == 0) { red[0][wave] = a; red[1][wave] = b; red[2][wave] = c; red[3][wave] = d; }
  __syncthreads();
  if (tid == 0) {
    for (int w = 1; w < 16; ++w) {
      if (PASS == 0) { a = fmin(a, red[0][w]); b = fmax(b, red[1][w]); c += red[2][w]; }
      else { a += red[0][w]; b += red[1][w]; c += red[2][w]; }
    }
    if (PASS == 0) { ws[0] = a; ws[1] = b; ws[2] = c; }
    else {
      const double var = a / (double)n;
      out6[0] = ws[0]; out6[1] = ws[1]; out6[2] = mean; out6[3] = var;
      out6[4] = b / pow(var, 1.5) / (double)n;
      out6[5] = c / (var * var) / (double)n - 3.0;
    }
  }
}
}

void tensor_moments(hipStream_t st, const float* base, long rows, int cols, long ld, double* out6, double* ws, int nb, int hf, int hi) {
  hipLaunchKernelGGL(tensor_moments_kernel<0>, dim3(1), dim3(1024), 0, st, base, rows, cols, ld, out6, ws, nb, hf, hi);
  hipLaunchKernelGGL(tensor_moments_kernel<1>, dim3(1), dim3(1024), 0, st, base, rows, cols, ld, out6, ws, nb, hf, hi);
  check_launch("tensor_moments");
}

}
```

### eesen_amd/csrc/rec_plan.cpp

```cpp
#include "rec_kernels.h"

#include <atomic>
#include <map>
#include <mutex>
#include <tuple>

namespace eesen {
namespace {

constexpr int NW = kRecWaves;

std::atomic<int> g_share_override{0};
int gpu_share() {
  static const int env = [] { const char* e = getenv("EESEN_GPU_SHARE"); const int v = e && *e ? atoi(e) : 0; return v < 1 ? 0 : v; }();
  if (env) return env;
  const int o = g_share_override.load(std::memory_order_relaxed);
  return o > 0 ? o : 1;
}
int share_of_cus() {
  int ncu = 256, dev = 0;
  (void)hipGetDevice(&dev);
  (void)hipDeviceGetAttribute(&ncu, hipDeviceAttributeMultiprocessorCount, dev);
  return std::max(1, ncu / gpu_share());
}

template <class... Args>
void plan_launch(hipStream_t st, const void* fn, int wgs, Args... args) {
  void* argv[] = {static_cast<void*>(&args)...};
  EESEN_HIP_CHECK(hipLaunchKernel(fn, dim3(wgs), dim3(NW * 64), argv, 0, st));
}

bool bf_census(const RecKernel& k, int wgs) {
  static std::mutex mu;
  static std::map<std::tuple<int, const void*, int>, bool> seen;
  int dev = 0;
  if (hipGetDevice(&dev) != hipSuccess) return false;
  if (gpu_share() > 1) return false;
  std::lock_guard<std::mutex> lock(mu);
  const auto key = std::make_tuple(dev, k.fn, wgs);
  if (auto it = seen.find(key); it != seen.end()) return it->second;
  bool ok = false;
  unsigned* w = nullptr;
  if (hipDeviceSynchronize() == hipSuccess && hipMalloc(reinterpret_cast<void**>(&w), 2 * sizeof(unsigned)) == hipSuccess) {
    for (int take = 0; take < 3 && !ok; ++take) {
      if (hipMemset(w, 0, 2 * sizeof(unsigned)) != hipSuccess) break;
      LstmLayerDev L{};
      L.T = -1;
      unsigned* err = w + 1;
      int spin_limit = 0;
      unsigned long long* trace = nullptr;
      RecRole role{1, 1, 1, 0};
      void* argv[] = {&L, &w, &err, &spin_limit, &trace, &role};
      if (hipLaunchKernel(k.fn, dim3(wgs), dim3(NW * 64), argv, 0, nullptr) != hipSuccess) { (void)hipGetLastError(); break; }
      unsigned e = 1;
      ok = hipMemcpy(&e, w + 1, sizeof(unsigned), hipMemcpyDeviceToHost) == hipSuccess && e == 0;
    }
    (void)hipFree(w);
  }
  seen[key] = ok;
  if (getenv("EESEN_PRINT_PLAN")) fprintf(stderr, "LOG (eesen_hip) residency census: %d workgroups of %s on device %d: %s\n", wgs, k.name, dev, ok ? "seen co-resident" : "NOT seen");
  return ok;
}

bool fits(const RecKernel& k, dim3 grid, bool census = false) {
  int dev = 0, ncu = 0, nb = 0;
  if (hipGetDevice(&dev) != hipSuccess) return false;
  if (hipDeviceGetAttribute(&ncu, hipDeviceAttributeMultiprocessorCount, dev) != hipSuccess) return false;
  {
    static std::mutex mu;
    static std::map<std::pair<int, const void*>, int> cache;
    std::lock_guard<std::mutex> lock(mu);
    const auto key = std::make_pair(dev, k.fn);
    auto it = cache.find(key);
    if (it == cache.end()) {
      if (hipOccupancyMaxActiveBlocksPerMultiprocessor(&nb, k.fn, NW * 64, 0) != hipSuccess) return false;
      it = cache.emplace(key, nb).first;
    }
    nb = it->second;
  }
  const long wgs = (long)grid.x * grid.y * grid.z;
  if (wgs <= (long)ncu * std::max(1, nb - 1) / gpu_share()) return true;
  return census && wgs <= (long)ncu * nb / gpu_share() && bf_census(k, (int)wgs);
}


size_t ctl_words(size_t groups) { return groups * kShards * kShardStride; }

bool line_aligned(int seqs, int cols) { return ((size_t)seqs * cols * sizeof(float)) % 128 == 0; }

template <class F>
int pick_windows(int S, int seq_tile, F fits_with) {
  for (int nwin = 1; nwin <= 8; nwin *= 2) {
    if (S % nwin != 0 || (S / nwin) % seq_tile != 0) { if (nwin == 1 && fits_with(S)) return 1; continue; }
    if (fits_with(S / nwin)) return nwin;
  }
  return 0;
}

void take(RecPlan& P, const RecKernel& k, const dim3& grid, size_t words, int seq_tile, int units, int windows) {
  P.kind = k.kind; P.fn = k.fn; P.kernel = k.name;
  P.seq_tile = seq_tile; P.units = units; P.windows = windows; P.ctl_words = words;
  P.grid[0] = (int)grid.x; P.grid[1] = (int)grid.y; P.grid[2] = (int)grid.z;
  P.wgs = (int)(grid.x * grid.y * grid.z);
  P.wgs_per_cu = std::max(1, cdiv(P.wgs, share_of_cus()));
  static std::mutex mu;
  static std::map<const void*, std::pair<int, int>> cache;
  std::lock_guard<std::mutex> lock(mu);
  auto it = cache.find(P.fn);
  if (it == cache.end()) {
    hipFuncAttributes a{};
    if (hipFuncGetAttributes(&a, P.fn) != hipSuccess) { (void)hipGetLastError(); return; }
    it = cache.emplace(P.fn, std::make_pair((int)a.numRegs, (int)a.sharedSizeBytes)).first;
  }
  P.vgprs = it->second.first;
  P.lds = it->second.second;
  if (P.vgprs > 0) P.free_vgprs = 512 - P.wgs_per_cu * (NW / 4) * ((P.vgprs + 7) & ~7);
}

struct FwdTile { int mt, nt; };
struct BfPlan { bool on; int cpw, nt, ap, wp; bool f16; };

bool small_xchg(const LstmLayerDev& L, int bytes_per_unit_row) {
  return (size_t)L.T * L.ndir * cdiv(L.S, 16) * (size_t)(L.H / 32) * bytes_per_unit_row < ((size_t)1 << 31);
}
bool bf_fits(const LstmLayerDev& L, const BfPlan& P, int Sw) {
  const RecKernel* k = rec_kernel(kFwdBf, P.cpw, P.nt, P.ap, P.wp, P.f16);
  return k && fits(*k, dim3(L.H / (4 * P.nt), L.ndir, cdiv(Sw, 16)),  true);
}
bool narrow2_ok(const LstmLayerDev& L, int need) {
  const bool f16 = L.fwd_f16 && L.wm_amax != nullptr;
  if (!L.fwd_narrow2 || !(L.fwd_split || f16) || L.fwd_bf16 || L.X == nullptr || L.drop_mode || L.T < 2 || L.H % 32 != 0) return false;
  if (!small_xchg(L, 1024 * 3)) return false;
  return bf_fits(L, f16 ? BfPlan{true, need, 2, 2, 2, true} : BfPlan{true, need, 2, 3, 3, false}, L.S);
}
FwdTile fwd_tile(const LstmLayerDev& L) {
  const int need = ((L.H + 31) / 32 + NW - 1) / NW;
  const int ncu = share_of_cus();
  const bool t16_ok = L.H % 8 == 0 && (L.S > 16 || need > 2 || (L.fwd_t16_small && L.fwd_split && !L.drop_mode && L.X && L.H % 32 == 0));
  const long narrow_wgs = (long)(L.H / 8) * L.ndir * cdiv(L.S, 16);
  const bool narrow_full = narrow_wgs > ncu && !(narrow_wgs <= 2L * ncu && need <= 2 && narrow2_ok(L, need));
  if (t16_ok && L.H % 16 == 0 && need <= 4 && (need > 2 || narrow_full)) return {1, 4};
  if (t16_ok && need <= 2) return {1, 2};
  return {2, 1};
}

BfPlan bf_plan_shape(const LstmLayerDev& L, const FwdTile& ft) {
  const BfPlan off{false, 0, 0, 0, 0, false};
  if (L.X == nullptr || L.drop_mode || L.T < 2 || L.H % 32 != 0) return off;
  if (L.fwd_bf16) {
    if (L.H % 256 != 0 || L.H / 256 > 4 || !small_xchg(L, 1024)) return off;
    return {true, L.H / 256, 4, 1, 2, false};
  }
  const bool f16 = L.fwd_f16 && L.wm_amax != nullptr;
  if (L.fwd_split || f16) {
    const int need = (L.H / 32 + NW - 1) / NW;
    if (f16 && ft.mt == 1 && ft.nt == 4 && L.H % 256 == 0 && L.H / 256 <= 4 && small_xchg(L, 1024 * 2)) return {true, L.H / 256, 4, 2, 2, true};
    if (ft.mt != 1 || ft.nt != 2 || need > 2 || L.H % 8 != 0 || !small_xchg(L, 1024 * 3)) return off;
    if (f16) return {true, need, 2, 2, 2, true};
    if (L.fwd_split) return {true, need, 2, 3, 3, false};
  }
  return off;
}

bool bwd_ksplit_shape(const LstmLayerDev& L, int stile) {
  return L.bwd_ksplit && stile == 16 && !L.drop_mode && L.H % 256 == 0 && L.H >= 768 && L.H <= 1024 && L.T >= 2;
}
bool bwd_planes_shape(const LstmLayerDev& L, int stile) {
  const int cpw = L.H / (32 * NW);
  return L.bwd_f16 && L.wm_amax != nullptr && bwd_ksplit_shape(L, stile) && (cpw == 2 || cpw == 4) && L.H % (32 * NW) == 0;
}

}

void set_gpu_share(int n) { g_share_override.store(n < 1 ? 1 : n, std::memory_order_relaxed); }
int gpu_share_value() { return gpu_share(); }

float handoff_flight_ns() {
  static float cache[64] = {0};
  static std::mutex mu;
  std::lock_guard<std::mutex> lock(mu);
  int dev = 0;
  if (hipGetDevice(&dev) != hipSuccess || dev < 0 || dev >= 64) return 0.f;
  if (cache[dev] > 0.f) return cache[dev];
  unsigned* flags = nullptr;
  unsigned long long* out = nullptr;
  EESEN_HIP_CHECK(hipMalloc(reinterpret_cast<void**>(&flags), 64 * sizeof(unsigned)));
  EESEN_HIP_CHECK(hipMalloc(reinterpret_cast<void**>(&out), sizeof(unsigned long long)));
  int rounds = 2000;
  double ns[5];
  for (int rep = 0; rep < 5; ++rep) {
    EESEN_HIP_CHECK(hipMemset(flags, 0, 64 * sizeof(unsigned)));
    void* argv[] = {&flags, &out, &rounds};
    (void)hipLaunchKernel(handoff_pingpong_fn(), dim3(2), dim3(64), argv, 0, nullptr);
    unsigned long long ticks = 0;
    EESEN_HIP_CHECK(hipMemcpy(&ticks, out, sizeof(ticks), hipMemcpyDeviceToHost));
    ns[rep] = ticks ? 10.0 * (double)ticks / (2.0 * rounds) : 500.0;
  }
  std::sort(ns, ns + 5);
  (void)hipFree(flags);
  (void)hipFree(out);
  cache[dev] = (float)std::min(2000.0, std::max(100.0, ns[2]));
  return cache[dev];
}

void wait_for_word(hipStream_t st, const unsigned* word, unsigned target, unsigned* err, double limit_s) {
  unsigned long long ticks = (unsigned long long)(std::max(0.05, limit_s) * 1e8);
  void* argv[] = {&word, &target, &err, &ticks};
  (void)hipLaunchKernel(wait_for_word_fn(), dim3(1), dim3(64), argv, 0, st);
  check_launch("wait_for_word");
}

RecPlan lstm_fwd_plan(const LstmLayerDev& L) {
  RecPlan P;
  const int need = ((L.H + 31) / 32 + NW - 1) / NW;
  const FwdTile ft = fwd_tile(L);
  if (need > 4 || (ft.nt == 2 && need > 2) || L.H % (4 * ft.nt) != 0 || L.T < 2) return P;
  if (!line_aligned(L.S, L.ndir * L.H)) return P;
  if ((size_t)(L.T + 2) * L.S * L.ndir * L.H * sizeof(float) >= ((size_t)1 << 31)) return P;
  BfPlan B = bf_plan_shape(L, ft);
  const bool drop = L.drop_mode != 0;
  const int cpw32 = ft.nt == 2 ? std::min(need, 2) : need <= 2 ? need : 4;
  int nwin = B.on ? pick_windows(L.S, 16, [&](int Sw) { return bf_fits(L, B, Sw); }) : 0;
  if (nwin == 0) {
    B.on = false;
    const RecKernel* probe = rec_kernel(kFwdF32, cpw32, ft.mt, ft.nt, drop, false);
    nwin = pick_windows(L.S, 16 * ft.mt, [&](int Sw) { return probe && fits(*probe, dim3(L.H / (4 * ft.nt), L.ndir, cdiv(Sw, 16 * ft.mt))); });
  }
  if (nwin == 0) return P;
  if (nwin > 1 && !line_aligned(L.S / nwin, L.ndir * L.H)) return P;
  const int mt = B.on ? 1 : ft.mt, nt = B.on ? B.nt : ft.nt, nz = cdiv(L.S, 16 * mt);
  auto answer = [&](const RecKernel& k, const dim3& grid, size_t words, int seq_tile, int windows, bool one_window) {
    take(P, k, grid, words, seq_tile, 4 * nt, windows);
    P.seq_tiles = nz;
    P.one_window = one_window;
    P.leaves_room = nt <= 2 && (!B.on || (long)(L.H / (4 * nt)) * L.ndir * nz <= share_of_cus());
    P.bf16 = L.fwd_bf16 && k.kind == kRecFwdBf;
  };
  const dim3 grid(L.H / (4 * nt), L.ndir, cdiv(L.S / nwin, 16 * mt));
  const size_t words = ctl_words(grid.y * grid.z);
  if (B.on) {
    if (words <= (size_t)kCtlHalf) answer(*rec_kernel(kFwdBf, B.cpw, B.nt, B.ap, B.wp, B.f16), grid, words, 16, nwin, nwin == 1);
    return P;
  }
  const bool xchg = L.X != nullptr && ft.mt == 1 && L.H % 32 == 0 && !drop && small_xchg(L, 2048);
  if (L.fwd_mux && nwin == 2 && ft.mt == 1 && ft.nt == 4 && need > 2 && need <= 4 && !drop && L.H % 32 == 0) {
    const RecKernel& k = *rec_kernel(kFwdMux, 4, 4, xchg);
    const dim3 mgrid(L.H / 16, L.ndir, cdiv(nz, 2));
    if (fits(k, mgrid) && ctl_words((size_t)L.ndir * nz) <= (size_t)kCtlHalf) {
      answer(k, mgrid, ctl_words((size_t)L.ndir * nz), 32, 1, false);
      return P;
    }
  }
  if (words > (size_t)kCtlHalf) return P;
  const RecKernel* k = rec_kernel(kFwdF32, cpw32, ft.mt, ft.nt, drop, xchg);
  EESEN_REQUIRE(k != nullptr, EESEN_ERR_STATE, "no instantiation of the fp32 forward tile for this plan");
  answer(*k, grid, words, 16 * ft.mt, nwin, nwin == 1);
  return P;
}

void lstm_fwd_launch(hipStream_t st, const RecPlan& P, const LstmLayerDev& L0, unsigned* cnt, unsigned* err, int spin_limit,
                     unsigned long long* trace, hipEvent_t after_reset) {
  EESEN_REQUIRE(P.kind == kRecFwdBf || P.kind == kRecFwdMux || P.kind == kRecFwdF32, EESEN_ERR_STATE, "not a forward recurrence plan");
  const RecRole role{P.grid[0], P.grid[1], P.grid[2], L0.xcd_map};
  for (int w = 0; w < P.windows; ++w) {
    LstmLayerDev L = L0;
    if (P.kind == kRecFwdMux) { L.s_begin = 0; L.s_count = 0; }
    else { L.s_count = L0.S / P.windows; L.s_begin = w * L.s_count; }
    if (P.kind != kRecFwdMux && P.wgs_per_cu >= 2 && !L0.poll_raw) L.poll_delay = L0.poll_delay * 7 / 4;
    EESEN_HIP_CHECK(hipMemsetAsync(cnt, 0, sizeof(unsigned) * P.ctl_words, st));
    if (after_reset && P.one_window) EESEN_HIP_CHECK(hipEventRecord(after_reset, st));
    if (P.kind == kRecFwdMux) plan_launch(st, P.fn, P.wgs, L, cnt, err, spin_limit, role);
    else plan_launch(st, P.fn, P.wgs, L, cnt, err, spin_limit, trace, role);
  }
}

RecPlan lstm_bwd_plan(const LstmLayerDev& L) {
  RecPlan P;
  const int need = ((4 * L.H + 31) / 32 + NW - 1) / NW;
  const int ldG = L.ndir * 4 * L.H;
  const long blocks16 = (long)cdiv(L.H, 16) * L.ndir * cdiv(L.S, 16);
  const int stile = 2 * blocks16 <= share_of_cus() && L.S > 8 ? 8 : 16;
  P.light = stile == 8;
  if (need > 16 || L.T < 2) return P;
  if (!line_aligned(L.S, ldG)) return P;
  const size_t blk_bytes = (size_t)L.S * ldG * sizeof(float);
  const long max_blocks = (long)((((size_t)1 << 31) - 1) / blk_bytes);
  if (max_blocks < 3) return P;
  int chunk = (int)std::min<long>(L.T, max_blocks - 1);
  if (chunk < L.T) { int p2 = 1; while (p2 * 2 <= chunk) p2 *= 2; chunk = p2; }
  P.chunk = chunk;
  auto in_windows = [&](const RecKernel* k, int gx, int seq_tile, int units, int quarters) {
    if (!k) return false;
    auto grid_of = [&](int Sw) { return dim3(gx, L.ndir, cdiv(Sw, seq_tile)); };
    auto words_of = [&](const dim3& g) { return ctl_words((size_t)g.y * g.z * quarters); };
    const int nwin = pick_windows(L.S, seq_tile, [&](int Sw) { return words_of(grid_of(Sw)) <= (size_t)kCtlHalf && fits(*k, grid_of(Sw)); });
    if (nwin == 0 || (nwin > 1 && !line_aligned(L.S / nwin, ldG))) return false;
    take(P, *k, grid_of(L.S / nwin), words_of(grid_of(L.S / nwin)), seq_tile, units, nwin);
    return true;
  };
  for (int pass = 0; pass < 2; ++pass) {
    const int stq = (L.bwd_q4_st8 == 2) == (pass == 0) ? 8 : 4;
    if (!L.bwd_q4 || L.drop_mode || L.H % 32 != 0 || L.H > 512 || chunk < L.T) break;
    if (stq == 4 && stile != 8) continue;
    if (stq == 8 && !(L.bwd_q4_st8 && L.S > 8)) continue;
    const int cpw = 2 * ((L.H + 127) / 128);
    const dim3 grid(L.H / 32, L.ndir, cdiv(L.S, stq));
    const size_t words = ctl_words((size_t)grid.y * grid.z);
    const RecKernel& k = *rec_kernel(kBwdQ4, cpw, stq);
    if (fits(k, grid) && words <= (size_t)kCtlHalf) {
      take(P, k, grid, words, stq, 32, 1);
      return P;
    }
  }
  if (bwd_ksplit_shape(L, stile)) {
    const int cpw = L.H / (32 * NW), gx = L.H / 64 * 4;
    const size_t px = (size_t)2 * L.ndir * cdiv(L.S, 16) * (size_t)(L.H / 64) * 4096 * 2;
    if (bwd_planes_shape(L, stile) && in_windows(rec_kernel(kBwdKsplitH, cpw), gx, 16, 64, 4)) {
      P.need_px = px; P.need_dgh = true;
      P.need_ex = (size_t)L.T * L.ndir * cdiv(L.S, 16) * (size_t)(L.H / 16) * 16;
      return P;
    }
    const RecKernel* k = rec_kernel(kBwdKsplit, cpw);
    const int nwin = !k ? 0 : pick_windows(L.S, 16, [&](int Sw) {
      const dim3 grid(gx, L.ndir, cdiv(Sw, 16));
      return ctl_words((size_t)grid.y * grid.z * 4) <= (size_t)kCtlHalf && fits(*k, grid);
    });
    if (nwin == 2 && L.bwd_mux && cpw >= 2 && cpw <= 4) {
      const int nz = cdiv(L.S, 16);
      const dim3 grid(gx, L.ndir, cdiv(nz, 2));
      const size_t words = ctl_words((size_t)L.ndir * nz * 4);
      const RecKernel& km = *rec_kernel(kBwdKsplitMux, cpw);
      if (words <= (size_t)kCtlHalf && fits(km, grid)) {
        take(P, km, grid, words, 32, 64, 1);
        P.need_px = px;
        return P;
      }
    }
    if (nwin > 0 && (nwin == 1 || line_aligned(L.S / nwin, ldG))) {
      const dim3 grid(gx, L.ndir, cdiv(L.S / nwin, 16));
      take(P, *k, grid, ctl_words((size_t)grid.y * grid.z * 4), 16, 64, nwin);
      P.need_px = px;
      return P;
    }
  }
  in_windows(rec_kernel(kBwdGeneric, need <= 1 ? 1 : need <= 2 ? 2 : need <= 4 ? 4 : need <= 8 ? 8 : 16, stile, L.drop_mode != 0), cdiv(L.H, 16), stile, 16, 1);
  return P;
}

void lstm_bwd_launch(hipStream_t st, const RecPlan& P, const LstmLayerDev& L0, const float* dY, int lddy, float* DG, unsigned* cnt,
                     unsigned* err, int spin_limit, unsigned long long* trace) {
  EESEN_REQUIRE(P.kind == kRecBwdQ4 || P.kind == kRecBwdKsplit || P.kind == kRecBwdKsplitMux || P.kind == kRecBwdGeneric, EESEN_ERR_STATE, "not a backward recurrence plan");
  EESEN_REQUIRE(!P.need_px || (L0.PX && L0.px_floats >= P.need_px), EESEN_ERR_STATE, "the backward plan's partial-sum exchange space (RecPlan::need_px) was not handed over");
  EESEN_REQUIRE(!P.need_dgh || (L0.DGH && L0.EX), EESEN_ERR_STATE, "the backward plan's plane and exponent buffers (RecPlan::need_dgh, need_ex) were not handed over");
  const RecRole role{P.grid[0], P.grid[1], P.grid[2], L0.xcd_map};
  const bool whole_batch = P.kind == kRecBwdQ4 || P.kind == kRecBwdKsplitMux;
  unsigned long long* px = reinterpret_cast<unsigned long long*>(L0.PX);
  int chunk = P.chunk;
  for (int w = 0; w < P.windows; ++w) {
    LstmLayerDev L = L0;
    if (whole_batch) { L.s_begin = 0; L.s_count = 0; }
    else { L.s_count = L0.S / P.windows; L.s_begin = w * L.s_count; }
    EESEN_HIP_CHECK(hipMemsetAsync(cnt, 0, sizeof(unsigned) * P.ctl_words, st));
    if (P.need_px) EESEN_HIP_CHECK(hipMemsetAsync(L.PX, 0, sizeof(float) * P.need_px, st));
    if (P.kind == kRecBwdQ4) plan_launch(st, P.fn, P.wgs, L, dY, lddy, DG, cnt, err, spin_limit, trace, role);
    else if (P.kind == kRecBwdKsplitMux) plan_launch(st, P.fn, P.wgs, L, dY, lddy, DG, px, cnt, err, spin_limit, role, chunk);
    else if (P.kind == kRecBwdKsplit) plan_launch(st, P.fn, P.wgs, L, dY, lddy, DG, px, cnt, err, spin_limit, role, chunk, trace);
    else plan_launch(st, P.fn, P.wgs, L, dY, lddy, DG, cnt, err, spin_limit, trace, role, chunk);
  }
}

}
```

### eesen_amd/csrc/tuning.h

```cpp
#pragma once
#include <cstdlib>

namespace eesen {

struct Tuning {
  int persistent = 1;
  int overlap = -1, gate_fwd = -1, side_lds_kb = -1;
  int spin_limit = 400000;
  bool spin_limit_set = false;
  int bwd_q4 = 1, bwd_q4_st8 = 1, fwd_narrow2 = 1, fwd_t16_small = 1, bwd_ksplit = 1, fwd_mux = 1, bwd_mux = 1, xcd_map = 1, fwd_mid = 1, fwd_split = 1, fwd_f16 = 1, bwd_f16 = 1;
  int comm_defer = -1;
  int trace = 0;
  bool print_flight = false;
  const char* poll_ns = nullptr;

  static Tuning from_env() {
    Tuning t;
    auto num = [](const char* name, int dflt) {
      const char* e = getenv(name);
      return e && *e ? atoi(e) : dflt;
    };
    t.persistent = num("EESEN_PERSISTENT", 1);
    t.overlap = num("EESEN_OVERLAP", -1);
    t.gate_fwd = num("EESEN_GATE_FWD", -1);
    t.fwd_mid = num("EESEN_FWD_MID", 1);
    t.side_lds_kb = num("EESEN_SIDE_LDS_KB", -1);
    t.spin_limit_set = getenv("EESEN_SPIN_LIMIT") != nullptr;
    t.spin_limit = num("EESEN_SPIN_LIMIT", 400000);
    t.bwd_q4 = num("EESEN_BWD_Q4", 1);
    t.bwd_q4_st8 = num("EESEN_BWD_Q4_ST8", 1);
    t.fwd_narrow2 = num("EESEN_FWD_NARROW2", 1);
    t.fwd_t16_small = num("EESEN_FWD_T16_SMALL", 1);
    t.bwd_ksplit = num("EESEN_BWD_KSPLIT", 1);
    t.fwd_mux = num("EESEN_FWD_MUX", 1);
    t.bwd_mux = num("EESEN_BWD_MUX", 1);
    t.fwd_split = num("EESEN_FWD_SPLIT", 1);
    t.fwd_f16 = num("EESEN_FWD_F16", 1);
    t.bwd_f16 = num("EESEN_BWD_F16", 1);
    t.xcd_map = num("EESEN_XCD_MAP", 1);
    t.comm_defer = num("EESEN_COMM_DEFER", -1);
    t.trace = num("EESEN_TRACE", 0);
    t.print_flight = getenv("EESEN_PRINT_FLIGHT") != nullptr;
    t.poll_ns = getenv("EESEN_POLL_NS");
    return t;
  }
};

}
```

Baseline: 999,900.

## Batch per-step memsets, SGD updates and weight-derived refreshes into few kernels

Adds a step_prep kernel that zeroes all LSTM boundary states, milestone words and per-layer recurrence counters in one launch, so the persistent launches skip their own counter memsets. Per-layer SGD updates become one multi-segment kernel that also zeroes the derived amax area. A single weights_refresh kernel recomputes the transposed recurrent weights and the row/column amax bounds for all layers. The aim is to cut the many small launches and memsets per training step. In exchange, counter and amax buffers are laid out per layer, and correctness now depends on the clean-state bookkeeping.

```diff
diff --git a/eesen_amd/csrc/kernels.h b/eesen_amd/csrc/kernels.h
--- a/eesen_amd/csrc/kernels.h
+++ b/eesen_amd/csrc/kernels.h
@@ -104,9 +104,9 @@
 RecPlan lstm_fwd_plan(const LstmLayerDev& L);
 RecPlan lstm_bwd_plan(const LstmLayerDev& L);
 void lstm_fwd_launch(hipStream_t st, const RecPlan& plan, const LstmLayerDev& L, unsigned* cnt, unsigned* err, int spin_limit,
-                     unsigned long long* trace = nullptr, hipEvent_t after_reset = nullptr);
+                     unsigned long long* trace = nullptr, hipEvent_t after_reset = nullptr, bool counters_clean = false);
 void lstm_bwd_launch(hipStream_t st, const RecPlan& plan, const LstmLayerDev& L, const float* dY, int lddy, float* DG, unsigned* cnt,
-                     unsigned* err, int spin_limit, unsigned long long* trace = nullptr);
+                     unsigned* err, int spin_limit, unsigned long long* trace = nullptr, bool counters_clean = false);
 void lstm_bias_peep_grads(hipStream_t st, const LstmLayerDev& L, const float* DG, float* bias_grad, float* peep_grad,
                           float* ws, size_t ws_floats);
 size_t lstm_bias_peep_ws_floats(int T, int S, int H, int ndir);
@@ -155,6 +155,28 @@
 
 void sgd_update(hipStream_t st, float* param, float* corr, const float* fresh, long n, float mmt, float lr_coef,
                 float max_grad, const unsigned* skip = nullptr, const float* live = nullptr);
+struct SgdSeg {
+  size_t off;
+  long n;
+  float lr_coef, max_grad;
+};
+void sgd_update_multi(hipStream_t st, float* param, float* corr, const float* fresh, const SgdSeg* segs, int nsegs, float mmt,
+                      const unsigned* skip, const float* live, unsigned* zero, size_t zero_words);
+struct RefreshLayer {
+  const float* wm = nullptr;
+  float* wmT = nullptr;
+  unsigned* wm_amax = nullptr;
+  int H = 0, ndir = 0;
+  const float* w = nullptr;
+  unsigned *w_rows = nullptr, *w_cols = nullptr;
+  int rows = 0, cols = 0;
+};
+void weights_refresh(hipStream_t st, const RefreshLayer* layers, int nlayers);
+struct PrepSeg {
+  unsigned* p;
+  size_t words;
+};
+void step_prep(hipStream_t st, const PrepSeg* segs, int nsegs);
 void zero_if_set(hipStream_t st, float* p, long n, const unsigned* word);
 void adaptive_update(hipStream_t st, float* param, float* corr, const float* fresh, float* accu, long n, float mmt, float lr,
                      float max_grad, float eps, float rho, float one_minus_rho, bool rmsprop, const unsigned* skip = nullptr,
diff --git a/eesen_amd/csrc/net.cpp b/eesen_amd/csrc/net.cpp
--- a/eesen_amd/csrc/net.cpp
+++ b/eesen_amd/csrc/net.cpp
@@ -297,7 +297,28 @@
   if (tn.overlap < 0)
     for (const Layer& L : layers)
       if (L.is_lstm() && L.H > 512) overlap = false;
-  amax.reserve(1 + layers.size());
+  {
+    size_t n = 1 + ((layers.size() + 3) & ~(size_t)3) + 3;
+    std::vector<size_t> at(layers.size(), 0);
+    for (size_t li = 0; li < layers.size(); ++li) {
+      const Layer& L = layers[li];
+      if (!L.trainable()) continue;
+      at[li] = n;
+      n += (size_t)pad4(L.is_lstm() ? L.ndir * 4 * L.H : L.dout) + (size_t)pad4(L.din);
+    }
+    amax.reserve(n);
+    derived_words = n - 1;
+    for (size_t li = 0; li < layers.size(); ++li)
+      if (Layer& L = layers[li]; L.trainable()) {
+        L.bw_rows = amax.p + at[li];
+        L.bw_cols = L.bw_rows + pad4(L.is_lstm() ? L.ndir * 4 * L.H : L.dout);
+      }
+  }
+  cnt.reserve((size_t)2 * layers.size() * kCtlHalf);
+  EESEN_HIP_CHECK(hipMemsetAsync(cnt.p, 0, cnt.cap * sizeof(unsigned), st));
+  cnt_clean.assign(2 * layers.size(), 0);
+  mile.reserve(32 * layers.size());
+  EESEN_HIP_CHECK(hipMemsetAsync(mile.p, 0, mile.cap * sizeof(unsigned), st));
   EESEN_HIP_CHECK(hipMemsetAsync(amax.p, 0, amax.cap * sizeof(float), st));
   EESEN_HIP_CHECK(hipMemsetD32Async(reinterpret_cast<hipDeviceptr_t>(amax.p), 0x3f800000, 1, st));
   finalized = true;
@@ -308,8 +329,11 @@
 void Net::measure(const float* Pm, long nrows, int cols, int ld, DevBuf<float>& out_rows, DevBuf<float>& out_cols) {
   out_rows.reserve((size_t)nrows);
   out_cols.reserve((size_t)cols);
+  measure(Pm, nrows, cols, ld, out_rows.p, out_cols.p);
+}
+void Net::measure(const float* Pm, long nrows, int cols, int ld, float* out_rows, float* out_cols) {
   amax_ws.reserve((size_t)kAmaxBlocks * std::min(16384, (cols + 3) & ~3));
-  amax_rows_cols(st, Pm, nrows, cols, ld, out_rows.p, out_cols.p, amax_ws.p);
+  amax_rows_cols(st, Pm, nrows, cols, ld, out_rows, out_cols, amax_ws.p);
 }
 bool Net::x_is_bounded(int li) const {
   if (li == 0) return false;
@@ -324,9 +348,9 @@
   for (size_t li = 0; li < layers.size(); ++li) {
     Layer& L = layers[li];
     if (L.is_lstm()) {
-      if (need_w) measure(params.p + L.p_off + L.off_wx, (long)L.ndir * 4 * L.H, pad4(L.din), pad4(L.din), L.bw.rows, L.bw.cols);
+      if (need_w) measure(params.p + L.p_off + L.off_wx, (long)L.ndir * 4 * L.H, pad4(L.din), pad4(L.din), L.bw_rows, L.bw_cols);
       if (!wm_valid) amax_abs_accumulate(st, params.p + L.p_off + L.off_wm, (long)L.ndir * 4 * L.H, L.H, L.H, am_wm((int)li));
-    } else if (L.kind == EESEN_LAYER_AFFINE && need_w) measure(params.p + L.p_off + L.off_w, L.dout, pad4(L.din), pad4(L.din), L.bw.rows, L.bw.cols);
+    } else if (L.kind == EESEN_LAYER_AFFINE && need_w) measure(params.p + L.p_off + L.off_w, L.dout, pad4(L.din), pad4(L.din), L.bw_rows, L.bw_cols);
   }
   wm_valid = true;
   if (mode2) wamax_valid = true;
@@ -345,8 +369,32 @@
   accu_init = true;
 }
 
-void Net::refresh_derived() {
+void Net::refresh_derived(bool zeroed) {
   wamax_valid = wm_valid = false;
+  if (tn.step_prep) {
+    const bool mode2 = gemm_mode() == 2;
+    if (!zeroed) EESEN_HIP_CHECK(hipMemsetAsync(amax.p + 1, 0, derived_words * sizeof(float), st));
+    std::vector<RefreshLayer> jobs;
+    for (size_t li = 0; li < layers.size(); ++li) {
+      Layer& L = layers[li];
+      if (!L.trainable()) continue;
+      RefreshLayer j;
+      if (L.is_lstm()) {
+        j.wm = params.p + L.p_off + L.off_wm; j.wmT = L.WmT.p; j.wm_amax = reinterpret_cast<unsigned*>(am_wm((int)li));
+        j.H = L.H; j.ndir = L.ndir;
+      }
+      if (mode2) {
+        j.w = params.p + L.p_off + (L.is_lstm() ? L.off_wx : L.off_w);
+        j.rows = L.is_lstm() ? L.ndir * 4 * L.H : L.dout; j.cols = pad4(L.din);
+        j.w_rows = reinterpret_cast<unsigned*>(L.bw_rows); j.w_cols = reinterpret_cast<unsigned*>(L.bw_cols);
+      }
+      jobs.push_back(j);
+    }
+    weights_refresh(st, jobs.data(), (int)jobs.size());
+    wm_valid = true;
+    wamax_valid = mode2;
+    return;
+  }
   for (Layer& L : layers)
     if (L.is_lstm())
       for (int dir = 0; dir < L.ndir; ++dir)
@@ -601,10 +649,42 @@
   forward_pass();
 }
 
+static void reserve_lstm(Net& net, Layer& L) {
+  const int H = L.H, nd = L.ndir, T = net.T, S = net.S;
+  L.G.reserve((size_t)net.rows * nd * 4 * H);
+  const size_t state = (size_t)(T + 2) * S * nd * H;
+  L.C.reserve(state);
+  L.Y.reserve(state);
+  if (net.persistent && H % 32 == 0) L.X.reserve((size_t)T * nd * ((S + 15) / 16) * (size_t)(H / 32) * 768);
+}
+
+void Net::step_prep_launch() {
+  std::vector<PrepSeg> segs;
+  for (Layer& L : layers)
+    if (L.is_lstm()) reserve_lstm(*this, L);
+  const std::vector<RecPlan> bwd = bwd_plans(T);
+  for (size_t li = 0; li < layers.size(); ++li) {
+    Layer& L = layers[li];
+    if (!L.is_lstm()) continue;
+    const size_t blk = (size_t)S * L.ndir * L.H, last = (size_t)(T + 1) * blk;
+    for (float* p : {L.C.p, L.Y.p, L.C.p + last, L.Y.p + last}) segs.push_back(PrepSeg{reinterpret_cast<unsigned*>(p), blk});
+    segs.push_back(PrepSeg{mile.p + 32 * li, 2});
+    const RecPlan fp = persistent ? lstm_fwd_plan(lstm_view(*this, L, T)) : RecPlan{};
+    const RecPlan* plans[2] = {&fp, &bwd[li]};
+    for (int pass = 0; pass < 2; ++pass) {
+      const size_t words = plans[pass]->kind != kRecNone ? plans[pass]->ctl_words : 0;
+      if (words) segs.push_back(PrepSeg{cnt_region((int)li, pass), words});
+      cnt_clean[2 * li + pass] = words;
+    }
+  }
+  step_prep(st, segs.data(), (int)segs.size());
+}
+
 void Net::forward_pass() {
   const float* x = input.p;
   int ldx = pad4(layers[0].din);
   ++steps_since_clean;
+  if (tn.step_prep) step_prep_launch();
   info_fwd_persistent = info_lstm_layers = info_fwd_bf16 = 0;
   bool g_gated = false;
   int gated_rows = 0;
@@ -618,20 +698,18 @@
     if (half && L.trainable()) {
       if (x_is_bounded(li_)) x_amax = bound_one();
       else { measure(x, rows, L.din, ldx, L.bx.rows, L.bx.cols); x_amax = GemmBound{L.bx.rows.p, 1}; }
-      w_amax = GemmBound{L.bw.rows.p, 1};
+      w_amax = GemmBound{L.bw_rows, 1};
     }
     if (L.is_lstm()) {
       const int H = L.H, nd = L.ndir, ldY = nd * H, ldG = nd * 4 * H;
-      L.G.reserve((size_t)rows * ldG);
-      const size_t state = (size_t)(T + 2) * S * ldY;
-      L.C.reserve(state);
-      L.Y.reserve(state);
-      if (persistent && H % 32 == 0) L.X.reserve((size_t)T * nd * ((S + 15) / 16) * (size_t)(H / 32) * 768);
-      const size_t blk = (size_t)S * ldY * sizeof(float);
-      EESEN_HIP_CHECK(hipMemsetAsync(L.C.p, 0, blk, st));
-      EESEN_HIP_CHECK(hipMemsetAsync(L.Y.p, 0, blk, st));
-      EESEN_HIP_CHECK(hipMemsetAsync(L.C.p + (size_t)(T + 1) * S * ldY, 0, blk, st));
-      EESEN_HIP_CHECK(hipMemsetAsync(L.Y.p + (size_t)(T + 1) * S * ldY, 0, blk, st));
+      if (!tn.step_prep) {
+        reserve_lstm(*this, L);
+        const size_t blk = (size_t)S * ldY * sizeof(float);
+        EESEN_HIP_CHECK(hipMemsetAsync(L.C.p, 0, blk, st));
+        EESEN_HIP_CHECK(hipMemsetAsync(L.Y.p, 0, blk, st));
+        EESEN_HIP_CHECK(hipMemsetAsync(L.C.p + (size_t)(T + 1) * S * ldY, 0, blk, st));
+        EESEN_HIP_CHECK(hipMemsetAsync(L.Y.p + (size_t)(T + 1) * S * ldY, 0, blk, st));
+      }
       prepare_dropout(*this, L);
       if (g_gated) {
         if (gated_rows < rows) {
@@ -671,14 +749,16 @@
       { const int ti_ = timer.begin(st, 1);
       v.poll_delay = delay_fwd;
       v.poll_raw = poll_raw;
+      unsigned* const mile_l = mile.p + 32 * li_;
+      unsigned* const cnt_f = cnt_region(li_, 0);
       if (plan_mid) {
-        mile.reserve(32);
-        EESEN_HIP_CHECK(hipMemsetAsync(mile.p, 0, 2 * sizeof(unsigned), st));
+        if (!tn.step_prep) EESEN_HIP_CHECK(hipMemsetAsync(mile_l, 0, 2 * sizeof(unsigned), st));
         EESEN_HIP_CHECK(hipEventRecord(ev_gate_reset, st));
-        v.milestone = mile.p;
+        v.milestone = mile_l;
         v.milestone_step = mile_step;
       }
-      if (pers) lstm_fwd_launch(st, fp, v, ctl.p, ctl.p + kCtlWords - 1, spin_limit, trace.p, plan_gate ? ev_gate_reset.get() : nullptr);
+      if (pers) lstm_fwd_launch(st, fp, v, cnt_f, ctl.p + kCtlWords - 1, spin_limit, trace.p, plan_gate ? ev_gate_reset.get() : nullptr,
+                                take_clean(li_, 0, fp.ctl_words));
       else
         for (int step = 0; step < T; ++step) lstm_fwd_step(st, v, step);
       info_fwd_persistent += pers ? 1 : 0;
@@ -691,16 +771,16 @@
         nxt->G.reserve((size_t)rows * ldG2);
         EESEN_HIP_CHECK(hipStreamWaitEvent(st2, ev_gate_reset, 0));
         const int tj_ = timer.begin(st2, 0);
-        GemmGate gate{ctl.p, ctl.p + kCtlWords - 1, nd, fp.seq_tiles, fp.grid[0], T, S, spin_limit};
+        GemmGate gate{cnt_f, ctl.p + kCtlWords - 1, nd, fp.seq_tiles, fp.grid[0], T, S, spin_limit};
         gated_rows = rows / 128 * 128;
         gemm_f32_nt_gated(st2, gated_rows, ldG2, ldY, L.Y.p + (size_t)S * ldY, ldY, params.p + nxt->p_off + nxt->off_wx, pad4(nxt->din),
-                          nxt->G.p, ldG2, params.p + nxt->p_off + nxt->off_bias, gate, half ? bound_one() : GemmBound{}, half ? GemmBound{nxt->bw.rows.p, 1} : GemmBound{});
+                          nxt->G.p, ldG2, params.p + nxt->p_off + nxt->off_bias, gate, half ? bound_one() : GemmBound{}, half ? GemmBound{nxt->bw_rows, 1} : GemmBound{});
         timer.end(st2, tj_);
         EESEN_HIP_CHECK(hipEventRecord(ev_gate_done, st2));
         g_gated = true;
       }
       if (plan_mid) {
-        EESEN_HIP_CHECK(hipMemsetD32Async(reinterpret_cast<hipDeviceptr_t>(mile.p + 1), 1, 1, st));
+        EESEN_HIP_CHECK(hipMemsetD32Async(reinterpret_cast<hipDeviceptr_t>(mile_l + 1), 1, 1, st));
         const int ldG2 = nxt->ndir * 4 * nxt->H;
         nxt->G.reserve((size_t)rows * ldG2);
         mid_r0 = ((T - 1 - mile_step) * S + 255) / 256 * 256;
@@ -710,12 +790,12 @@
       if (plan_mid && mid_r1 > mid_r0) {
         const int ldG2 = nxt->ndir * 4 * nxt->H;
         EESEN_HIP_CHECK(hipStreamWaitEvent(st2, ev_gate_reset, 0));
-        wait_for_word(st2, mile.p + 1, 1u, ctl.p + kCtlWords - 1, 2.0 * std::max(1.0, T / 1000.0) * std::max(1.0, spin_limit / 400000.0));
+        wait_for_word(st2, mile_l + 1, 1u, ctl.p + kCtlWords - 1, 2.0 * std::max(1.0, T / 1000.0) * std::max(1.0, spin_limit / 400000.0));
         const int tj_ = timer.begin(st2, 0);
         gemm_f32(st2, true, true, mid_r1 - mid_r0, ldG2, nxt->din, 1.f, L.Y.p + (size_t)S * ldY + (size_t)mid_r0 * ldY, ldY,
                  params.p + nxt->p_off + nxt->off_wx, pad4(nxt->din), 0.f, nxt->G.p + (size_t)mid_r0 * ldG2, ldG2,
                  params.p + nxt->p_off + nxt->off_bias, nullptr, 0,  64, fwd_bf16,
-                 half ? bound_one() : GemmBound{}, half ? GemmBound{nxt->bw.rows.p, 1} : GemmBound{});
+                 half ? bound_one() : GemmBound{}, half ? GemmBound{nxt->bw_rows, 1} : GemmBound{});
         timer.end(st2, tj_);
         EESEN_HIP_CHECK(hipEventRecord(ev_gate_done, st2));
       } }
@@ -857,7 +937,7 @@
       if (want_in) {
         if (ld_n != L.din) EESEN_HIP_CHECK(hipMemsetAsync(dn, 0, (size_t)rows * ld_n * sizeof(float), st));
         gemm_f32(st, true, false, rows, L.din, L.dout, 1.f, d, ld_d, params.p + L.p_off + L.off_w, pad4(L.din), 0.f, dn, ld_n,
-                 nullptr, nullptr, 0, 0, false, half ? GemmBound{L.bd.rows.p, 1} : GemmBound{}, half ? GemmBound{L.bw.cols.p, 1} : GemmBound{});
+                 nullptr, nullptr, 0, 0, false, half ? GemmBound{L.bd.rows.p, 1} : GemmBound{}, half ? GemmBound{L.bw_cols, 1} : GemmBound{});
       }
       gemm_f32(st, false, false, L.dout, L.din, rows, 1.f, d, ld_d, x, ldx, 0.f, fr + L.off_w, pad4(L.din), nullptr, ws.p, ws_floats, 0, false,
                half ? GemmBound{L.bd.cols.p, 1} : GemmBound{}, x_cols(li));
@@ -886,7 +966,8 @@
       }
       { const int ti_ = timer.begin(st, 3);
       if (bp.kind != kRecNone) {
-        lstm_bwd_launch(st, bp, v, d, ld_d, DGl, ctl.p + kCtlHalf, ctl.p + kCtlWords - 1, spin_limit, trace.p ? trace.p + 640 : nullptr);
+        lstm_bwd_launch(st, bp, v, d, ld_d, DGl, cnt_region(li, 1), ctl.p + kCtlWords - 1, spin_limit, trace.p ? trace.p + 640 : nullptr,
+                        take_clean(li, 1, bp.ctl_words));
         ++info_bwd_persistent;
       } else
         for (int step = 0; step < T; ++step) lstm_bwd_step(st, v, step, d, ld_d, DGl, DCF.p);
@@ -898,7 +979,7 @@
         const int ti_ = timer.begin(st, 4);
         if (ld_n != L.din) EESEN_HIP_CHECK(hipMemsetAsync(dn, 0, (size_t)rows * ld_n * sizeof(float), st));
         gemm_f32(st, true, false, rows, L.din, ldG, 1.f, DGl, ldG, params.p + L.p_off + L.off_wx, pad4(L.din), 0.f, dn, ld_n,
-                 nullptr, nullptr, 0, 0, false, half ? GemmBound{L.bd.rows.p, 1} : GemmBound{}, half ? GemmBound{L.bw.cols.p, 1} : GemmBound{});
+                 nullptr, nullptr, 0, 0, false, half ? GemmBound{L.bd.rows.p, 1} : GemmBound{}, half ? GemmBound{L.bw_cols, 1} : GemmBound{});
         timer.end(st, ti_);
         EESEN_HIP_CHECK(hipEventRecord(ev_rec, st));
       }
@@ -999,6 +1080,8 @@
   const float* live = comm && live_valid ? fresh.p + P : nullptr;
   comm_check_alive(comm);
   { const int ti_ = timer.begin(st, 5);
+  const bool multi = tn.step_prep && rule == 0;
+  std::vector<SgdSeg> segs;
   for (int li = (int)layers.size() - 1; li >= 0; --li) {
     Layer& L = layers[li];
     if (L.p_n) {
@@ -1008,7 +1091,9 @@
         timer.end(st, tw_);
         bucket_pending[li] = 0;
       }
-      if (rule == 0) {
+      if (multi) {
+        segs.push_back(SgdSeg{L.p_off, (long)L.p_n, lr * L.coef, L.max_grad});
+      } else if (rule == 0) {
         sgd_update(st, params.p + L.p_off, corr.p + L.p_off, fresh.p + L.p_off, (long)L.p_n, mmt, lr * L.coef, L.max_grad, skip, live);
       } else {
         init_accu();
@@ -1017,7 +1102,10 @@
       }
     }
   }
-  refresh_derived();
+  if (multi)
+    sgd_update_multi(st, params.p, corr.p, fresh.p, segs.data(), (int)segs.size(), mmt, skip, live, reinterpret_cast<unsigned*>(amax.p + 1),
+                     derived_words);
+  refresh_derived(multi);
   timer.end(st, ti_); }
   grads_sanitized = false;
   live_valid = false;
diff --git a/eesen_amd/csrc/net.h b/eesen_amd/csrc/net.h
--- a/eesen_amd/csrc/net.h
+++ b/eesen_amd/csrc/net.h
@@ -10,7 +10,7 @@
 namespace eesen {
 
 inline int pad4(int x) { return (x + 3) & ~3; }
-constexpr size_t kCtlWords = 2 * kCtlHalf + 32;
+constexpr size_t kCtlWords = 32;
 
 struct Layer {
   int kind = 0, din = 0, dout = 0;
@@ -26,7 +26,8 @@
   DevBuf<float> X;
   size_t off_w = 0, off_b = 0;
   DevBuf<float> out;
-  struct Bounds { DevBuf<float> rows, cols; } bw, bx, bd;
+  struct Bounds { DevBuf<float> rows, cols; } bx, bd;
+  float *bw_rows = nullptr, *bw_cols = nullptr;
   float drop[9] = {0, 0, 0, 0, 0, 0, 0, 0, 0};
   bool has_dropout() const { return drop[0] > 0.f || drop[5] != 0.f || drop[6] != 0.f; }
   DevBuf<float> fmask;
@@ -119,6 +120,16 @@
   bool fwd_bf16_rec = false;
   int info_fwd_bf16 = 0;
   DevBuf<unsigned> ctl;
+  DevBuf<unsigned> cnt;
+  std::vector<size_t> cnt_clean;
+  unsigned* cnt_region(int li, int pass) { return cnt.p + ((size_t)2 * li + pass) * kCtlHalf; }
+  bool take_clean(int li, int pass, size_t words) {
+    size_t& c = cnt_clean[(size_t)2 * li + pass];
+    const bool clean = words > 0 && c >= words;
+    c = 0;
+    return clean;
+  }
+  void step_prep_launch();
   Tuning tn;
   int persistent = 1;
   int info_fwd_persistent = 0, info_bwd_persistent = 0, info_lstm_layers = 0;
@@ -142,12 +153,14 @@
   void get_dropout_masks(int layer, float* fwd_host, float* rec_host, int* info4);
   size_t ws_floats = 0;
   DevBuf<float> amax, amax_ws;
+  size_t derived_words = 0;
   bool wamax_valid = false, wm_valid = false;
   bool amx_valid = false;
   float* am_wm(int li) { return amax.p + 1 + li; }
   GemmBound bound_one() const { return GemmBound{amax.p, 0}; }
   bool x_is_bounded(int li) const;
   void measure(const float* P, long rows, int cols, int ld, DevBuf<float>& out_rows, DevBuf<float>& out_cols);
+  void measure(const float* P, long rows, int cols, int ld, float* out_rows, float* out_cols);
   void ensure_weight_amax();
   PhaseTimer timer;
   Comm* comm = nullptr;
@@ -189,7 +202,7 @@
   void backpropagate(const float* out_diff, int ldd, float* in_diff, int ldi);
   void backpropagate_impl(const float* out_diff, int ldd, float* in_diff, int ldi);
   void update();
-  void refresh_derived();
+  void refresh_derived(bool zeroed = false);
   int tensor_moments(int which, int layer, double* out6_host, int cap_tensors);
   void read(const std::string& path);
   void write(const std::string& path, bool binary);
diff --git a/eesen_amd/csrc/optim.hip b/eesen_amd/csrc/optim.hip
--- a/eesen_amd/csrc/optim.hip
+++ b/eesen_amd/csrc/optim.hip
@@ -30,6 +30,158 @@
     corr[i] = c;
     param[i] -= lr_coef * c;
   }
+}
+
+constexpr int kSgdSegs = 16;
+struct SgdSegTable {
+  SgdSeg s[kSgdSegs];
+};
+__global__ __launch_bounds__(256) void sgd_update_multi_kernel(float* __restrict__ param_, float* __restrict__ corr_,
+                                                               const float* __restrict__ fresh_, SgdSegTable tab, float mmt,
+                                                               const unsigned* __restrict__ skip, const float* __restrict__ live,
+                                                               unsigned* __restrict__ zero, size_t zero_words) {
+  const long stride = (long)gridDim.x * blockDim.x;
+  if (blockIdx.y == 0)
+    for (size_t i = (size_t)blockIdx.x * blockDim.x + threadIdx.x; i < zero_words; i += (size_t)stride) zero[i] = 0u;
+  if (skip && *skip) return;
+  if (live && *live == 0.f) return;
+  const SgdSeg sg = tab.s[blockIdx.y];
+  float* __restrict__ param = param_ + sg.off;
+  float* __restrict__ corr = corr_ + sg.off;
+  const float* __restrict__ fresh = fresh_ + sg.off;
+  const long n = sg.n;
+  const float lr_coef = sg.lr_coef, max_grad = sg.max_grad;
+  const long n4 = n >> 2;
+  for (long i = (long)blockIdx.x * blockDim.x + threadIdx.x; i < n4; i += stride) {
+    float4 p = reinterpret_cast<float4*>(param)[i];
+    float4 c = reinterpret_cast<float4*>(corr)[i];
+    const float4 g = reinterpret_cast<const float4*>(fresh)[i];
+    c.x = mmt * c.x + g.x; c.y = mmt * c.y + g.y; c.z = mmt * c.z + g.z; c.w = mmt * c.w + g.w;
+    if (max_grad > 0.f) {
+      c.x = fminf(fmaxf(c.x, -max_grad), max_grad); c.y = fminf(fmaxf(c.y, -max_grad), max_grad);
+      c.z = fminf(fmaxf(c.z, -max_grad), max_grad); c.w = fminf(fmaxf(c.w, -max_grad), max_grad);
+    }
+    p.x -= lr_coef * c.x; p.y -= lr_coef * c.y; p.z -= lr_coef * c.z; p.w -= lr_coef * c.w;
+    reinterpret_cast<float4*>(corr)[i] = c;
+    reinterpret_cast<float4*>(param)[i] = p;
+  }
+  for (long i = (n4 << 2) + (long)blockIdx.x * blockDim.x + threadIdx.x; i < n; i += stride) {
+    float c = mmt * corr[i] + fresh[i];
+    if (max_grad > 0.f) c = fminf(fmaxf(c, -max_grad), max_grad);
+    corr[i] = c;
+    param[i] -= lr_coef * c;
+  }
+}
+
+constexpr int kPrepSegs = 56;
+struct PrepSegTable {
+  PrepSeg s[kPrepSegs];
+};
+__global__ __launch_bounds__(256) void step_prep_kernel(PrepSegTable tab) {
+  const PrepSeg sg = tab.s[blockIdx.y];
+  const size_t stride = (size_t)gridDim.x * blockDim.x, i0 = (size_t)blockIdx.x * blockDim.x + threadIdx.x;
+  if ((reinterpret_cast<uintptr_t>(sg.p) & 15) == 0 && (sg.words & 3) == 0) {
+    uint4* p4 = reinterpret_cast<uint4*>(sg.p);
+    for (size_t i = i0; i < sg.words / 4; i += stride) p4[i] = make_uint4(0u, 0u, 0u, 0u);
+  } else {
+    for (size_t i = i0; i < sg.words; i += stride) sg.p[i] = 0u;
+  }
+}
+
+constexpr int kRefreshLayers = 16, kRefreshStripRows = 64, kRefreshTiles = 4;
+struct RefreshTable {
+  RefreshLayer L[kRefreshLayers];
+  int first[kRefreshLayers + 1];
+  int tiles[kRefreshLayers];
+  int n;
+};
+__global__ __launch_bounds__(256) void weights_refresh_kernel(RefreshTable tab) {
+  __shared__ unsigned sh[32 * 33];
+  int k = 0;
+  while (k + 1 < tab.n && (int)blockIdx.x >= tab.first[k + 1]) ++k;
+  const RefreshLayer& L = tab.L[k];
+  int job = (int)blockIdx.x - tab.first[k];
+  const int tid = threadIdx.x, lane = tid & 63, wave = tid >> 6;
+  if (job < tab.tiles[k]) {
+    const int rows = 4 * L.H, cols = L.H;
+    const int tx_n = (cols + 32 * kRefreshTiles - 1) / (32 * kRefreshTiles), ty_n = (rows + 31) / 32;
+    const int dir = job / (tx_n * ty_n), t = job % (tx_n * ty_n);
+    const float* __restrict__ src = L.wm + (size_t)dir * rows * cols;
+    float* __restrict__ dst = L.wmT + (size_t)dir * rows * cols;
+    float(*tile)[33] = reinterpret_cast<float(*)[33]>(sh);
+    const int tx = tid & 31, ty = tid >> 5;
+    const int r0 = (t / tx_n) * 32;
+    unsigned m = 0u;
+    for (int q = 0; q < kRefreshTiles; ++q) {
+      const int c0 = ((t % tx_n) * kRefreshTiles + q) * 32;
+      if (c0 >= cols) break;
+#pragma unroll
+      for (int i = 0; i < 32; i += 8) {
+        const int r = r0 + ty + i, c = c0 + tx;
+        if (r < rows && c < cols) {
+          const float v = src[(size_t)r * cols + c];
+          tile[ty + i][tx] = v;
+          m = max(m, __builtin_bit_cast(unsigned, v) & 0x7fffffffu);
+        }
+      }
+      __syncthreads();
+#pragma unroll
+      for (int i = 0; i < 32; i += 8) {
+        const int c = c0 + ty + i, r = r0 + tx;
+        if (r < rows && c < cols) dst[(size_t)c * rows + r] = tile[tx][ty + i];
+      }
+      __syncthreads();
+    }
+#pragma unroll
+    for (int o = 32; o > 0; o >>= 1) m = max(m, (unsigned)__shfl_xor((int)m, o));
+    if (lane == 0) sh[wave] = m;
+    __syncthreads();
+    if (tid == 0) {
+      m = max(max(sh[0], sh[1]), max(sh[2], sh[3]));
+      if (m) atomicMax(L.wm_amax, m);
+    }
+    return;
+  }
+  job -= tab.tiles[k];
+  const int C = L.cols, nslab = (C + 1023) / 1024;
+  const int slab = job % nslab;
+  const long r0 = (long)(job / nslab) * kRefreshStripRows, r1 = min((long)L.rows, r0 + kRefreshStripRows);
+  for (int c = tid; c < 1024; c += 256) sh[c] = 0u;
+  __syncthreads();
+  const int c0 = slab * 1024 + lane * 4;
+  uint4 cm[4];
+#pragma unroll
+  for (int j = 0; j < 4; ++j) cm[j] = make_uint4(0u, 0u, 0u, 0u);
+  for (long r = r0 + wave; r < r1; r += 4) {
+    const float* row = L.w + r * C;
+    uint4 v[4];
+#pragma unroll
+    for (int j = 0; j < 4; ++j) {
+      const int c = c0 + 256 * j;
+      v[j] = c < C ? *reinterpret_cast<const uint4*>(row + c) : make_uint4(0u, 0u, 0u, 0u);
+    }
+    unsigned m = 0u;
+#pragma unroll
+    for (int j = 0; j < 4; ++j) {
+      v[j].x &= 0x7fffffffu; v[j].y &= 0x7fffffffu; v[j].z &= 0x7fffffffu; v[j].w &= 0x7fffffffu;
+      m = max(m, max(max(v[j].x, v[j].y), max(v[j].z, v[j].w)));
+      cm[j].x = max(cm[j].x, v[j].x); cm[j].y = max(cm[j].y, v[j].y); cm[j].z = max(cm[j].z, v[j].z); cm[j].w = max(cm[j].w, v[j].w);
+    }
+#pragma unroll
+    for (int o = 32; o > 0; o >>= 1) m = max(m, (unsigned)__shfl_xor((int)m, o));
+    if (lane == 0 && m) atomicMax(&L.w_rows[r], m);
+  }
+#pragma unroll
+  for (int j = 0; j < 4; ++j) {
+    const int c = lane * 4 + 256 * j;
+    if (cm[j].x) atomicMax(&sh[c], cm[j].x);
+    if (cm[j].y) atomicMax(&sh[c + 1], cm[j].y);
+    if (cm[j].z) atomicMax(&sh[c + 2], cm[j].z);
+    if (cm[j].w) atomicMax(&sh[c + 3], cm[j].w);
+  }
+  __syncthreads();
+  for (int c = tid; c < 1024; c += 256)
+    if (slab * 1024 + c < C && sh[c]) atomicMax(&L.w_cols[slab * 1024 + c], sh[c]);
 }
 
 __global__ __launch_bounds__(256) void adaptive_update_kernel(float* __restrict__ param, float* __restrict__ corr,
@@ -96,6 +248,59 @@
   check_launch("sgd_update");
 }
 
+void sgd_update_multi(hipStream_t st, float* param, float* corr, const float* fresh, const SgdSeg* segs, int nsegs, float mmt,
+                      const unsigned* skip, const float* live, unsigned* zero, size_t zero_words) {
+  for (int s0 = 0; s0 < nsegs || (s0 == 0 && zero_words); s0 += kSgdSegs) {
+    SgdSegTable tab{};
+    const int n = std::max(0, std::min(kSgdSegs, nsegs - s0));
+    long nmax = 0;
+    for (int k = 0; k < n; ++k) { tab.s[k] = segs[s0 + k]; nmax = std::max(nmax, segs[s0 + k].n); }
+    const int blocks = (int)std::min<long>(cdivl(nmax / 4 + 1, 256), 2048);
+    if (n == 0) {
+      tab.s[0] = SgdSeg{0, 0, 0.f, 0.f};
+    }
+    hipLaunchKernelGGL(sgd_update_multi_kernel, dim3(blocks, std::max(1, n)), dim3(256), 0, st, param, corr, fresh, tab, mmt, skip, live,
+                       s0 == 0 ? zero : nullptr, s0 == 0 ? zero_words : (size_t)0);
+    check_launch("sgd_update_multi");
+  }
+}
+
+void step_prep(hipStream_t st, const PrepSeg* segs, int nsegs) {
+  for (int s0 = 0; s0 < nsegs; s0 += kPrepSegs) {
+    PrepSegTable tab{};
+    const int n = std::min(kPrepSegs, nsegs - s0);
+    size_t wmax = 0;
+    for (int k = 0; k < n; ++k) { tab.s[k] = segs[s0 + k]; wmax = std::max(wmax, segs[s0 + k].words); }
+    const int blocks = (int)std::max<size_t>(1, std::min<size_t>((wmax / 4 + 1023) / 1024, 64));
+    hipLaunchKernelGGL(step_prep_kernel, dim3(blocks, n), dim3(256), 0, st, tab);
+    check_launch("step_prep");
+  }
+}
+
+void weights_refresh(hipStream_t st, const RefreshLayer* layers, int nlayers) {
+  for (int l0 = 0; l0 < nlayers; l0 += kRefreshLayers) {
+    RefreshTable tab{};
+    tab.n = std::min(kRefreshLayers, nlayers - l0);
+    long jobs = 0;
+    for (int k = 0; k < tab.n; ++k) {
+      const RefreshLayer& L = layers[l0 + k];
+      tab.L[k] = L;
+      tab.first[k] = (int)jobs;
+      tab.tiles[k] = L.wm ? L.ndir * cdiv(L.H, 32 * kRefreshTiles) * cdiv(4 * L.H, 32) : 0;
+      jobs += tab.tiles[k];
+      if (L.w) {
+        EESEN_REQUIRE(L.cols % 4 == 0 && (reinterpret_cast<uintptr_t>(L.w) & 15) == 0, EESEN_ERR_INVALID, "weights_refresh: rows of whole, aligned float4s");
+        jobs += (long)cdiv(L.rows, kRefreshStripRows) * cdiv(L.cols, 1024);
+      }
+      EESEN_REQUIRE(jobs < (1L << 30), EESEN_ERR_INVALID, "weights_refresh: too many jobs for one grid");
+    }
+    tab.first[tab.n] = (int)jobs;
+    if (jobs == 0) continue;
+    hipLaunchKernelGGL(weights_refresh_kernel, dim3((unsigned)jobs), dim3(256), 0, st, tab);
+    check_launch("weights_refresh");
+  }
+}
+
 void zero_if_set(hipStream_t st, float* p, long n, const unsigned* word) {
   if (n <= 0 || !word) return;
   hipLaunchKernelGGL(zero_if_set_kernel, dim3(256), dim3(256), 0, st, p, n, word);
diff --git a/eesen_amd/csrc/rec_plan.cpp b/eesen_amd/csrc/rec_plan.cpp
--- a/eesen_amd/csrc/rec_plan.cpp
+++ b/eesen_amd/csrc/rec_plan.cpp
@@ -259,7 +259,7 @@
 }
 
 void lstm_fwd_launch(hipStream_t st, const RecPlan& P, const LstmLayerDev& L0, unsigned* cnt, unsigned* err, int spin_limit,
-                     unsigned long long* trace, hipEvent_t after_reset) {
+                     unsigned long long* trace, hipEvent_t after_reset, bool counters_clean) {
   EESEN_REQUIRE(P.kind == kRecFwdBf || P.kind == kRecFwdMux || P.kind == kRecFwdF32, EESEN_ERR_STATE, "not a forward recurrence plan");
   const RecRole role{P.grid[0], P.grid[1], P.grid[2], L0.xcd_map};
   for (int w = 0; w < P.windows; ++w) {
@@ -267,7 +267,7 @@
     if (P.kind == kRecFwdMux) { L.s_begin = 0; L.s_count = 0; }
     else { L.s_count = L0.S / P.windows; L.s_begin = w * L.s_count; }
     if (P.kind != kRecFwdMux && P.wgs_per_cu >= 2 && !L0.poll_raw) L.poll_delay = L0.poll_delay * 7 / 4;
-    EESEN_HIP_CHECK(hipMemsetAsync(cnt, 0, sizeof(unsigned) * P.ctl_words, st));
+    if (w > 0 || !counters_clean) EESEN_HIP_CHECK(hipMemsetAsync(cnt, 0, sizeof(unsigned) * P.ctl_words, st));
     if (after_reset && P.one_window) EESEN_HIP_CHECK(hipEventRecord(after_reset, st));
     if (P.kind == kRecFwdMux) plan_launch(st, P.fn, P.wgs, L, cnt, err, spin_limit, role);
     else plan_launch(st, P.fn, P.wgs, L, cnt, err, spin_limit, trace, role);
@@ -348,7 +348,7 @@
 }
 
 void lstm_bwd_launch(hipStream_t st, const RecPlan& P, const LstmLayerDev& L0, const float* dY, int lddy, float* DG, unsigned* cnt,
-                     unsigned* err, int spin_limit, unsigned long long* trace) {
+                     unsigned* err, int spin_limit, unsigned long long* trace, bool counters_clean) {
   EESEN_REQUIRE(P.kind == kRecBwdQ4 || P.kind == kRecBwdKsplit || P.kind == kRecBwdKsplitMux || P.kind == kRecBwdGeneric, EESEN_ERR_STATE, "not a backward recurrence plan");
   EESEN_REQUIRE(!P.need_px || (L0.PX && L0.px_floats >= P.need_px), EESEN_ERR_STATE, "the backward plan's partial-sum exchange space (RecPlan::need_px) was not handed over");
   EESEN_REQUIRE(!P.need_dgh || (L0.DGH && L0.EX), EESEN_ERR_STATE, "the backward plan's plane and exponent buffers (RecPlan::need_dgh, need_ex) were not handed over");
@@ -360,7 +360,7 @@
     LstmLayerDev L = L0;
     if (whole_batch) { L.s_begin = 0; L.s_count = 0; }
     else { L.s_count = L0.S / P.windows; L.s_begin = w * L.s_count; }
-    EESEN_HIP_CHECK(hipMemsetAsync(cnt, 0, sizeof(unsigned) * P.ctl_words, st));
+    if (w > 0 || !counters_clean) EESEN_HIP_CHECK(hipMemsetAsync(cnt, 0, sizeof(unsigned) * P.ctl_words, st));
     if (P.need_px) EESEN_HIP_CHECK(hipMemsetAsync(L.PX, 0, sizeof(float) * P.need_px, st));
     if (P.kind == kRecBwdQ4) plan_launch(st, P.fn, P.wgs, L, dY, lddy, DG, cnt, err, spin_limit, trace, role);
     else if (P.kind == kRecBwdKsplitMux) plan_launch(st, P.fn, P.wgs, L, dY, lddy, DG, px, cnt, err, spin_limit, role, chunk);
diff --git a/eesen_amd/csrc/tuning.h b/eesen_amd/csrc/tuning.h
--- a/eesen_amd/csrc/tuning.h
+++ b/eesen_amd/csrc/tuning.h
@@ -8,7 +8,7 @@
   int overlap = -1, gate_fwd = -1, side_lds_kb = -1;
   int spin_limit = 400000;
   bool spin_limit_set = false;
-  int bwd_q4 = 1, bwd_q4_st8 = 1, fwd_narrow2 = 1, fwd_t16_small = 1, bwd_ksplit = 1, fwd_mux = 1, bwd_mux = 1, xcd_map = 1, fwd_mid = 1, fwd_split = 1, fwd_f16 = 1, bwd_f16 = 1;
+  int bwd_q4 = 1, bwd_q4_st8 = 1, fwd_narrow2 = 1, fwd_t16_small = 1, bwd_ksplit = 1, fwd_mux = 1, bwd_mux = 1, xcd_map = 1, fwd_mid = 1, fwd_split = 1, fwd_f16 = 1, bwd_f16 = 1, step_prep = 1;
   int comm_defer = -1;
   int trace = 0;
   bool print_flight = false;
@@ -38,6 +38,7 @@
     t.fwd_f16 = num("EESEN_FWD_F16", 1);
     t.bwd_f16 = num("EESEN_BWD_F16", 1);
     t.xcd_map = num("EESEN_XCD_MAP", 1);
+    t.step_prep = num("EESEN_STEP_PREP", 1);
     t.comm_defer = num("EESEN_COMM_DEFER", -1);
     t.trace = num("EESEN_TRACE", 0);
     t.print_flight = getenv("EESEN_PRINT_FLIGHT") != nullptr;
```

Result: no change. 1.001 million, median of 6 (+0.1%).
